# coolbeam/UPFlow_pytorch

Measured on AMD Instinct MI355X. Metric: frame-pairs/sec at 384x1280 bf16, higher is better.
Workload: dtype bf16; 1 GPU; config2: UPFlow_net inference forward (flow fwd+bwd, occlusion masks, SGU on), 384x1280, batch 4 per GPU, random-init weights; global_batch=4, parallelism=replicas x1 (image pairs sharded, no collective), ranks=1, hip_graph=True, capture_fallback=False, steps_in_flight=4, pyramid_convs=HIP (MFMA kernel), pyramid_dtype=fp16

## Files before the change

include/upflow_hip.h:

```cpp
#ifndef UPFLOW_HIP_H
#define UPFLOW_HIP_H

#ifdef __cplusplus
extern "C" {
#endif

enum { UPF_F32 = 0, UPF_F16 = 1, UPF_BF16 = 2 };
enum { UPF_OK = 0, UPF_EINVAL = -1, UPF_EDTYPE = -2, UPF_EALIGN = -3, UPF_EUNSUPPORTED = -4 };
enum { UPF_MASK_NONE = 0, UPF_MASK_LITERAL = 1, UPF_MASK_ROBUST = 2 };

const char* upf_version(void);
const char* upf_last_error(void);

int upf_corr81_forward(const void* f1, const void* f2, void* out,
                       int B, int C, int H, int W, int dtype,
                       long long out_batch_stride, float leaky_slope, void* stream);

int upf_corr81_forward_timed(const void* f1, const void* f2, void* out,
                             int B, int C, int H, int W, int dtype,
                             long long out_batch_stride, float leaky_slope, void* stream,
                             int nrep, float* avg_us, float* min_us);

int upf_corr81_norm_supported(int C, int dtype);
long long upf_corr81_norm_workspace_bytes(int B, int C, int H, int W);
int upf_corr81_norm_forward(const void* f1, const void* f2, void* out,
                            int B, int C, int H, int W, int dtype,
                            long long out_batch_stride, float leaky_slope, void* workspace, void* stream);
int upf_corr81_norm_forward_c8(const void* f1, const void* f2, void* out8, long long out8_batch_stride,
                               int B, int C, int H, int W, int dtype, float leaky_slope, void* workspace, void* stream);
int upf_corr81_norm_forward_pitched(const void* f1, const void* f2, int f_row_pitch, void* out,
                                    int B, int C, int H, int W, int dtype,
                                    long long out_batch_stride, float leaky_slope, void* workspace, void* stream);
int upf_corr81_norm_forward_c8_pitched(const void* f1, const void* f2, int f_row_pitch, void* out8, long long out8_batch_stride,
                                       int B, int C, int H, int W, int dtype, float leaky_slope, void* workspace, void* stream);
int upf_corr81_norm_forward_mixed(const void* f1, const void* f2, int f_row_pitch, void* out,
                                  int B, int C, int H, int W, int dtype, int out_dtype,
                                  long long out_batch_stride, float leaky_slope, void* workspace, void* stream);
int upf_corr81_norm_forward_c8_mixed(const void* f1, const void* f2, int f_row_pitch, void* out8, long long out8_batch_stride,
                                     int B, int C, int H, int W, int dtype, int out_dtype, float leaky_slope, void* workspace, void* stream);
int upf_corr81_norm_forward_timed(const void* f1, const void* f2, void* out,
                                  int B, int C, int H, int W, int dtype,
                                  long long out_batch_stride, float leaky_slope, void* workspace, void* stream,
                                  int nrep, float* avg_us, float* min_us);
int upf_corr81_norm_forward_c8_timed(const void* f1, const void* f2, void* out8, long long out8_batch_stride,
                                     int B, int C, int H, int W, int dtype, float leaky_slope, void* workspace, void* stream,
                                     int nrep, float* avg_us, float* min_us);

int upf_corr81_norm_forward_c8_timed_pitched(const void* f1, const void* f2, int f_row_pitch, void* out8, long long out8_batch_stride,
                                             int B, int C, int H, int W, int dtype, float leaky_slope, void* workspace, void* stream,
                                             int nrep, float* avg_us, float* min_us);

int upf_corr81_norm_forward_c8_timed_mixed(const void* f1, const void* f2, int f_row_pitch, void* out8, long long out8_batch_stride,
                                           int B, int C, int H, int W, int dtype, int out_dtype, float leaky_slope, void* workspace, void* stream,
                                           int nrep, float* avg_us, float* min_us);

int upf_corr_set_option(const char* name, int value);

int upf_corr81_backward(const void* f1, const void* f2, const void* grad_out, void* g1, void* g2,
                        int B, int C, int H, int W, int dtype, void* stream);

int upf_correlation_forward(const void* in1, const void* in2, void* out,
                            int B, int C, int H, int W, int dtype,
                            int pad_size, int kernel_size, int max_displacement,
                            int stride1, int stride2, int corr_type_multiply, void* stream);
int upf_correlation_backward(const void* in1, const void* in2, const void* grad_out, void* g1, void* g2,
                             int B, int C, int H, int W, int dtype,
                             int pad_size, int kernel_size, int max_displacement,
                             int stride1, int stride2, int corr_type_multiply, void* stream);
int upf_correlation_out_shape(int H, int W, int pad_size, int kernel_size, int max_displacement,
                              int stride1, int stride2, int* out_channels, int* out_h, int* out_w);

int upf_warp_forward(const void* x, const float* flow, void* y,
                     int B, int C, int H, int W, int dtype, int mask_mode, int batch_shift, void* stream);
int upf_warp_forward_strided(const void* x, long long x_batch_stride, const float* flow, void* y, long long y_batch_stride,
                             int B, int C, int H, int W, int dtype, int mask_mode, int batch_shift, void* stream);
int upf_warp_forward_pitched(const void* x, long long x_batch_stride, int x_row_pitch, const float* flow, void* y, long long y_batch_stride,
                             int y_row_pitch, int B, int C, int H, int W, int dtype, int mask_mode, int batch_shift, void* stream);
int upf_warp_forward_c8(const void* x8, long long x_batch_stride, const float* flow, void* y8, long long y_batch_stride,
                        int B, int n_oct, int H, int W, int dtype, int mask_mode, int batch_shift, void* stream);
long long upf_warp_backward_workspace_bytes(int B, int C, int H, int W);
int upf_warp_backward(const void* x, const float* flow, const void* grad_y,
                      void* gx, float* gflow, void* workspace,
                      int B, int C, int H, int W, int dtype, int mask_mode, int batch_shift, void* stream);

int upf_flow_upsample_forward(const float* x, float* y, int B, int C, int h, int w, int H, int W,
                              int if_rate, void* stream);
int upf_flow_upsample_backward(const float* grad_y, float* gx, int B, int C, int h, int w, int H, int W,
                               int if_rate, void* stream);

long long upf_sgu_blend_forward_workspace_bytes(int B, int h, int w, int Hf, int Wf);
int upf_sgu_blend_forward(const float* flow_init, const void* x_out, float* flow_up,
                          float* inter_flow, float* inter_mask, void* workspace,
                          int B, int h, int w, int Hf, int Wf, int dtype, void* stream);
int upf_sgu_blend_forward_flow16(const float* flow_init, const void* x_out, float* flow_up, void* flow16, long long flow16_batch_stride,
                                 int flow16_is_c8, int B, int H, int W, int dtype, void* stream);
long long upf_sgu_blend_backward_workspace_bytes(int B, int h, int w, int Hf, int Wf);
int upf_sgu_blend_backward(const float* flow_init, const void* x_out, const float* grad_flow_up,
                           float* g_flow_init32, float* g_x_out32, void* workspace,
                           int B, int h, int w, int Hf, int Wf, int dtype, void* stream);

long long upf_normalize_workspace_bytes(long long N, int HW);
int upf_normalize_forward(const void* x, void* y, float* mean, float* rstd, void* workspace,
                          long long N, int HW, int dtype, void* stream);
int upf_normalize_backward(const void* y, const void* grad_y, const float* rstd, void* gx,
                           long long N, int HW, int dtype, void* stream);

long long upf_conv_packed_bytes(int Cin, int Cout, int kernel_size);
int upf_conv_pack_weights(const void* w , void* w_packed, int Cin, int Cout, int kernel_size,
                          int dtype, void* stream);
int upf_conv_forward(const void* x, long long x_batch_stride, const void* w_packed, const float* bias,
                     void* y, long long y_batch_stride, int B, int Cin, int Cout, int H, int W,
                     int kernel_size, int dilation, int stride, float leaky_slope, int dtype, void* stream);
int upf_conv_forward_pitched(const void* x, long long x_batch_stride, int x_row_pitch, const void* w_packed, const float* bias,
                             void* y, long long y_batch_stride, int y_row_pitch, int B, int Cin, int Cout, int H, int W,
                             int kernel_size, int dilation, int stride, float leaky_slope, int dtype, void* stream);
int upf_conv1x1_forward_mixed(const void* x, long long x_batch_stride, int x_row_pitch, const void* w_packed, const float* bias,
                              void* y, long long y_batch_stride, int y_row_pitch, int y_is_c8, int B, int Cin, int Cout, int H, int W,
                              float leaky_slope, int dtype, int out_dtype, void* stream);
int upf_conv1x1_forward_c8_dual(const void* x, long long x_batch_stride, int x_row_pitch, const void* w_packed, const float* bias,
                                void* y8_a, long long ya_batch_stride, void* y8_b, long long yb_batch_stride,
                                int B, int Cin, int Cout, int H, int W, float leaky_slope, int dtype, int out_dtype, void* stream);
int upf_conv_set_option(const char* name, int value);

long long upf_conv_x3_packed_bytes(int Cin, int Cout, int kernel_size);
int upf_conv_x3_pack_weights(const float* w, void* w_packed, int Cin, int Cout, int kernel_size, void* stream);
int upf_conv_x3_forward(const float* x, long long x_batch_stride, const void* w_packed, const float* bias, float* y,
                        long long y_batch_stride, int B, int Cin, int Cout, int H, int W, int kernel_size, int dilation,
                        int stride, float leaky_slope, int nprod, void* stream);
int upf_conv_x3_set_option(const char* name, int value);
int upf_mfma_f16_denorm_probe(float* out_device, void* stream);

long long upf_conv_packed_bytes_k(int K, int Cout, int kernel_size);
int upf_conv_c8_k(int n8_oct, int C2);
int upf_conv_pack_weights_kmap(const void* w , void* w_packed, int Cin, int Cout, int kernel_size,
                               const int* kmap , int K, int dtype, void* stream);
int upf_conv_forward_c8(const void* x8, long long x8_batch_stride, int n8_oct, const void* x2, long long x2_batch_stride, int C2,
                        const void* w_packed, const float* bias, void* y, long long y_batch_stride, int y_is_c8,
                        int B, int Cout, int H, int W, int kernel_size, int dilation, int stride, float leaky_slope,
                        int dtype, void* stream);
int upf_conv_forward_c8_pitched(const void* x8, long long x8_batch_stride, int n8_oct, const void* x2, long long x2_batch_stride, int x2_row_pitch, int C2,
                                const void* w_packed, const float* bias, void* y, long long y_batch_stride, int y_row_pitch, int y_is_c8,
                                int B, int Cout, int H, int W, int kernel_size, int dilation, int stride, float leaky_slope,
                                int dtype, void* stream);
int upf_conv_c8_set_option(const char* name, int value);
long long upf_conv_packed_bytes_k16(int K, int Cout);
int upf_conv_pack_weights_kmap16(const void* w , void* w_packed, int Cin, int Cout,
                                 const int* kmap , int K, int dtype, void* stream);
int upf_conv_forward_c8_narrow(const void* x8, long long x8_batch_stride, int n8_oct, const void* w_packed16, const float* bias,
                               void* y, long long y_batch_stride, int y_is_c8, int B, int Cout, int H, int W, float leaky_slope,
                               int dtype, void* stream);
int upf_conv_forward_c8_split(const void* x8, long long x8_batch_stride, int n8_oct, const void* w_packed ,
                              const float* bias , void* y8, long long y_batch_stride, int C_main,
                              float* partial, long long partial_batch_stride , int partial_pitch ,
                              int B, int Cout, int H, int W, float leaky_slope, int dtype, void* stream);
int upf_conv_forward_c8_narrow_init(const void* x8, long long x8_batch_stride, int n8_oct, const void* w_packed16,
                                    const float* partial, long long partial_batch_stride, int partial_pitch, int partial_offset ,
                                    void* y, long long y_batch_stride, int y_is_c8, int B, int Cout, int H, int W, float leaky_slope,
                                    int dtype, void* stream);

int upf_conv_pair_forward(const void* x, long long x_batch_stride, int x_row_pitch, int Cin,
                          const void* wa_packed, const float* bias_a , float slope_a, int C1, int stride_a,
                          const void* wb_packed, const float* bias_b , float slope_b, int C2, int stride_b,
                          void* y, long long y_batch_stride, int y_row_pitch, int y_is_c8,
                          int B, int H, int W, int dtype, void* stream);

int upf_conv_pack_weights_f32(const float* w , void* w_packed, int Cin, int Cout, int kernel_size,
                              int dtype, int dgrad, void* stream);
int upf_conv_pack_weights_f32_multi(const float* const* w, void* const* w_packed, const int* Cin, const int* Cout, const int* kernel_size,
                                    const int* dgrad, int njobs, int dtype, void* stream);
int upf_conv_pack_stacked_dgrad(const float* const* w, const int* Cin, const int* Cout, const int* first_channel, int nlayers,
                                void* const* w_packed, const int* slice_channel, const int* slice_width, const int* nconsumers,
                                int nslices, int dtype, void* stream);
int upf_leaky_backward(const void* grad_y, const void* y, void* grad_pre, long long n, float slope, int dtype, void* stream);
int upf_conv_wgrad_supported(int Cin, int Cout, int H, int W, int kernel_size, int dilation, int stride, int dtype);
long long upf_conv_wgrad_workspace_bytes(int B, int Cin, int Cout, int H, int W, int kernel_size, int dilation);
int upf_conv_wgrad(const void* x, long long x_batch_stride, const void* grad_pre, long long g_batch_stride, float* grad_w,
                   void* workspace, int B, int Cin, int Cout, int H, int W, int kernel_size, int dilation, int dtype, void* stream);
typedef struct {
  const void* x;        long long x_batch_stride;
  const void* grad_pre; long long g_batch_stride;
  int B, H, W;
} upf_wgrad_level;
long long upf_conv_wgrad_multi_workspace_bytes(const upf_wgrad_level* levels, int nlevels, int Cin, int Cout, int kernel_size, int dilation);
int upf_conv_wgrad_multi(const upf_wgrad_level* levels , int nlevels, float* grad_w, void* workspace, int Cin, int Cout,
                         int kernel_size, int dilation, int dtype, void* stream);
int upf_conv_wgrad_multi_bias(const upf_wgrad_level* levels, int nlevels, float* grad_w, void* workspace, int Cin, int Cout,
                              int kernel_size, int dilation, const float* const* bias_partials , int npartials, float* grad_bias,
                              int dtype, void* stream);
int upf_space_to_depth2(const void* src, void* dst, int B, int C , int H, int W , int inverse, int dtype, void* stream);
int upf_conv_wgrad_s2d(const upf_wgrad_level* levels, int nlevels, float* grad_w, void* workspace, int Cin, int Cout, int dtype, void* stream);
int upf_act_grad(const void* src, long long src_batch_stride, const void* add, long long add_batch_stride, const void* y,
                 long long y_batch_stride, void* dst, long long dst_batch_stride, float* bias_partial, int B, int C, int HW,
                 float slope, int dtype, void* stream);
int upf_conv_forward_gated(const void* x, long long x_batch_stride, int x_row_pitch, const void* w_packed, const float* bias,
                           void* y, long long y_batch_stride, int y_row_pitch, const void* add, long long add_batch_stride,
                           const void* act, long long act_batch_stride, float mask_slope,
                           int B, int Cin, int Cout, int H, int W, int dtype, void* stream);
int upf_conv_bias_grad_finish(const float* const* partials , int npartials, float* grad_bias,
                              int Cout, void* stream);
long long upf_conv_bias_grad_workspace_bytes(int Cout);
int upf_conv_bias_grad(const void* grad_pre, long long g_batch_stride, float* grad_bias, void* workspace, int B, int Cout, int HW,
                       int dtype, void* stream);

int upf_flow_update(const float* a, const void* b, const void* c, void* out, long long out_batch_stride,
                    int out_is_f32, int N, int per_item, int dtype, void* stream);
int upf_flow_update_c8(const float* a, const void* b, const void* c, void* out8, long long out8_batch_stride,
                       int N, int HW, int dtype, void* stream);

int upf_occ_check(const float* flow_f, const float* flow_b, float* occ_fw, float* occ_bw,
                  int B, int H, int W, float alpha1, float alpha2, void* stream);

int upf_div_selftest(int size, unsigned long long* mismatches, void* stream);

int upf_census_forward(const float* gray1, const float* gray2, float* dist, int B, int H, int W, int max_distance, void* stream);
int upf_census_backward(const float* gray1, const float* gray2, const float* grad_dist, float* g_gray1, float* g_gray2,
                        int B, int H, int W, int max_distance, void* stream);

int upf_boundary_warp_forward(const float* image, const float* flow, const float* start, float* out,
                              int B, int C, int Hi, int Wi, int h, int w, void* stream);
int upf_boundary_warp_backward(const float* image, const float* flow, const float* start, const float* grad_out,
                               float* grad_flow, int B, int C, int Hi, int Wi, int h, int w, void* stream);

int upf_loss_partials(long long n_pixels);

int upf_robust_loss_forward(const float* x, const float* y, const float* occ, float* partials,
                            int B, int C, int HW, float eps, float q, void* stream);
int upf_robust_loss_backward(const float* x, const float* y, const float* occ, const float* coef,
                             float* grad_x, float* grad_y, int B, int C, int HW, float eps, float q, void* stream);

int upf_grey_forward(const float* image, float* grey, int B, int HW, void* stream);

int upf_msd_upup_partials(int B, int H, int W);
int upf_msd_upup_forward(const float* const* x_low, const int* hs, const int* ws, int nlevels, const float* y, const float* occ,
                         float* partials, float* out2, int B, int H, int W, float weight, float eps, float q, void* stream);
int upf_msd_upup_backward(const float* const* x_low, float* const* grad_x_low, const int* hs, const int* ws, int nlevels, const float* y,
                          const float* occ, const float* grad_out, const float* fwd_out2, int B, int H, int W, float weight, float eps, float q,
                          void* stream);

int upf_smooth_edge1_forward(const float* img, const float* pred, float* partials,
                             int B, int Ci, int Cp, int H, int W, void* stream);
int upf_smooth_edge1_backward(const float* img, const float* pred, const float* grad_up, float* grad_pred,
                              int B, int Ci, int Cp, int H, int W, void* stream);

#ifdef __cplusplus
}
#endif
#endif
```

upflow_pytorch_amd/_lib.py:

```python
import ctypes
import os

import torch

_PKG = os.path.dirname(os.path.abspath(__file__))
LIB_PATH = os.environ.get('UPF_HIP_LIB') or os.path.join(_PKG, 'libupflow_hip.so')

UPF_F32, UPF_F16, UPF_BF16 = 0, 1, 2
MASK_NONE, MASK_LITERAL, MASK_ROBUST = 0, 1, 2
_DTYPES = {torch.float32: UPF_F32, torch.float16: UPF_F16, torch.bfloat16: UPF_BF16}

_c = ctypes
_vp, _i, _f, _ll = _c.c_void_p, _c.c_int, _c.c_float, _c.c_longlong

SIGNATURES = {
    'upf_corr81_forward': [_vp, _vp, _vp, _i, _i, _i, _i, _i, _ll, _f, _vp],
    'upf_corr81_forward_timed': [_vp, _vp, _vp, _i, _i, _i, _i, _i, _ll, _f, _vp, _i, _c.POINTER(_f), _c.POINTER(_f)],
    'upf_corr81_norm_forward': [_vp, _vp, _vp, _i, _i, _i, _i, _i, _ll, _f, _vp, _vp],
    'upf_corr81_norm_forward_timed': [_vp, _vp, _vp, _i, _i, _i, _i, _i, _ll, _f, _vp, _vp, _i, _c.POINTER(_f), _c.POINTER(_f)],
    'upf_corr81_norm_forward_c8_timed': [_vp, _vp, _vp, _ll, _i, _i, _i, _i, _i, _f, _vp, _vp, _i, _c.POINTER(_f), _c.POINTER(_f)],
    'upf_corr81_norm_forward_pitched': [_vp, _vp, _i, _vp, _i, _i, _i, _i, _i, _ll, _f, _vp, _vp],
    'upf_corr81_norm_forward_c8_pitched': [_vp, _vp, _i, _vp, _ll, _i, _i, _i, _i, _i, _f, _vp, _vp],
    'upf_corr81_norm_forward_c8_timed_pitched': [_vp, _vp, _i, _vp, _ll, _i, _i, _i, _i, _i, _f, _vp, _vp, _i, _c.POINTER(_f), _c.POINTER(_f)],
    'upf_corr81_norm_forward_c8_timed_mixed': [_vp, _vp, _i, _vp, _ll, _i, _i, _i, _i, _i, _i, _f, _vp, _vp, _i, _c.POINTER(_f), _c.POINTER(_f)],
    'upf_warp_forward_pitched': [_vp, _ll, _i, _vp, _vp, _ll, _i, _i, _i, _i, _i, _i, _i, _i, _vp],
    'upf_conv_forward_gated': [_vp, _ll, _i, _vp, _vp, _vp, _ll, _i, _vp, _ll, _vp, _ll, _f, _i, _i, _i, _i, _i, _i, _vp],
    'upf_conv_forward_pitched': [_vp, _ll, _i, _vp, _vp, _vp, _ll, _i, _i, _i, _i, _i, _i, _i, _i, _i, _f, _i, _vp],
    'upf_conv_forward_c8_pitched': [_vp, _ll, _i, _vp, _ll, _i, _i, _vp, _vp, _vp, _ll, _i, _i, _i, _i, _i, _i, _i, _i, _i, _f, _i, _vp],
    'upf_corr81_norm_forward_mixed': [_vp, _vp, _i, _vp, _i, _i, _i, _i, _i, _i, _ll, _f, _vp, _vp],
    'upf_corr81_norm_forward_c8_mixed': [_vp, _vp, _i, _vp, _ll, _i, _i, _i, _i, _i, _i, _f, _vp, _vp],
    'upf_conv1x1_forward_mixed': [_vp, _ll, _i, _vp, _vp, _vp, _ll, _i, _i, _i, _i, _i, _i, _i, _f, _i, _i, _vp],
    'upf_conv1x1_forward_c8_dual': [_vp, _ll, _i, _vp, _vp, _vp, _ll, _vp, _ll, _i, _i, _i, _i, _i, _f, _i, _i, _vp],
    'upf_corr81_backward': [_vp, _vp, _vp, _vp, _vp, _i, _i, _i, _i, _i, _vp],
    'upf_correlation_forward': [_vp, _vp, _vp, _i, _i, _i, _i, _i, _i, _i, _i, _i, _i, _i, _vp],
    'upf_correlation_backward': [_vp, _vp, _vp, _vp, _vp, _i, _i, _i, _i, _i, _i, _i, _i, _i, _i, _i, _vp],
    'upf_correlation_out_shape': [_i, _i, _i, _i, _i, _i, _i, _c.POINTER(_i), _c.POINTER(_i), _c.POINTER(_i)],
    'upf_warp_forward': [_vp, _vp, _vp, _i, _i, _i, _i, _i, _i, _i, _vp],
    'upf_warp_forward_strided': [_vp, _ll, _vp, _vp, _ll, _i, _i, _i, _i, _i, _i, _i, _vp],
    'upf_warp_forward_c8': [_vp, _ll, _vp, _vp, _ll, _i, _i, _i, _i, _i, _i, _i, _vp],
    'upf_flow_update': [_vp, _vp, _vp, _vp, _ll, _i, _i, _i, _i, _vp],
    'upf_flow_update_c8': [_vp, _vp, _vp, _vp, _ll, _i, _i, _i, _vp],
    'upf_corr81_norm_forward_c8': [_vp, _vp, _vp, _ll, _i, _i, _i, _i, _i, _f, _vp, _vp],
    'upf_warp_backward': [_vp, _vp, _vp, _vp, _vp, _vp, _i, _i, _i, _i, _i, _i, _i, _vp],
    'upf_flow_upsample_forward': [_vp, _vp, _i, _i, _i, _i, _i, _i, _i, _vp],
    'upf_flow_upsample_backward': [_vp, _vp, _i, _i, _i, _i, _i, _i, _i, _vp],
    'upf_sgu_blend_forward': [_vp, _vp, _vp, _vp, _vp, _vp, _i, _i, _i, _i, _i, _i, _vp],
    'upf_sgu_blend_forward_flow16': [_vp, _vp, _vp, _vp, _ll, _i, _i, _i, _i, _i, _vp],
    'upf_sgu_blend_backward': [_vp, _vp, _vp, _vp, _vp, _vp, _i, _i, _i, _i, _i, _i, _vp],
    'upf_normalize_forward': [_vp, _vp, _vp, _vp, _vp, _ll, _i, _i, _vp],
    'upf_normalize_backward': [_vp, _vp, _vp, _vp, _ll, _i, _i, _vp],
    'upf_conv_pack_weights': [_vp, _vp, _i, _i, _i, _i, _vp],
    'upf_conv_forward': [_vp, _ll, _vp, _vp, _vp, _ll, _i, _i, _i, _i, _i, _i, _i, _i, _f, _i, _vp],
    'upf_conv_x3_pack_weights': [_vp, _vp, _i, _i, _i, _vp],
    'upf_conv_x3_forward': [_vp, _ll, _vp, _vp, _vp, _ll, _i, _i, _i, _i, _i, _i, _i, _i, _f, _i, _vp],
    'upf_mfma_f16_denorm_probe': [_vp, _vp],
    'upf_conv_pack_weights_f32': [_vp, _vp, _i, _i, _i, _i, _i, _vp],
    'upf_conv_pack_stacked_dgrad': [_c.POINTER(_vp), _c.POINTER(_i), _c.POINTER(_i), _c.POINTER(_i), _i, _c.POINTER(_vp), _c.POINTER(_i), _c.POINTER(_i), _c.POINTER(_i), _i, _i, _vp],
    'upf_conv_pack_weights_f32_multi': [_c.POINTER(_vp), _c.POINTER(_vp), _c.POINTER(_i), _c.POINTER(_i), _c.POINTER(_i), _c.POINTER(_i), _i, _i, _vp],
    'upf_conv_pack_weights_kmap': [_vp, _vp, _i, _i, _i, _vp, _i, _i, _vp],
    'upf_conv_forward_c8': [_vp, _ll, _i, _vp, _ll, _i, _vp, _vp, _vp, _ll, _i, _i, _i, _i, _i, _i, _i, _i, _f, _i, _vp],
    'upf_conv_pack_weights_kmap16': [_vp, _vp, _i, _i, _vp, _i, _i, _vp],
    'upf_conv_forward_c8_narrow': [_vp, _ll, _i, _vp, _vp, _vp, _ll, _i, _i, _i, _i, _i, _f, _i, _vp],
    'upf_conv_forward_c8_split': [_vp, _ll, _i, _vp, _vp, _vp, _ll, _i, _vp, _ll, _i, _i, _i, _i, _i, _f, _i, _vp],
    'upf_conv_forward_c8_narrow_init': [_vp, _ll, _i, _vp, _vp, _ll, _i, _i, _vp, _ll, _i, _i, _i, _i, _i, _f, _i, _vp],
    'upf_conv_pair_forward': [_vp, _ll, _i, _i, _vp, _vp, _f, _i, _i, _vp, _vp, _f, _i, _i, _vp, _ll, _i, _i, _i, _i, _i, _i, _vp],
    'upf_leaky_backward': [_vp, _vp, _vp, _ll, _f, _i, _vp],
    'upf_conv_wgrad': [_vp, _ll, _vp, _ll, _vp, _vp, _i, _i, _i, _i, _i, _i, _i, _i, _vp],
    'upf_conv_bias_grad': [_vp, _ll, _vp, _vp, _i, _i, _i, _i, _vp],
    'upf_conv_wgrad_multi': [_vp, _i, _vp, _vp, _i, _i, _i, _i, _i, _vp],
    'upf_conv_wgrad_multi_bias': [_vp, _i, _vp, _vp, _i, _i, _i, _i, _vp, _i, _vp, _i, _vp],
    'upf_space_to_depth2': [_vp, _vp, _i, _i, _i, _i, _i, _i, _vp],
    'upf_conv_wgrad_s2d': [_vp, _i, _vp, _vp, _i, _i, _i, _vp],
    'upf_act_grad': [_vp, _ll, _vp, _ll, _vp, _ll, _vp, _ll, _vp, _i, _i, _i, _f, _i, _vp],
    'upf_conv_bias_grad_finish': [_vp, _i, _vp, _i, _vp],
    'upf_census_forward': [_vp, _vp, _vp, _i, _i, _i, _i, _vp],
    'upf_census_backward': [_vp, _vp, _vp, _vp, _vp, _i, _i, _i, _i, _vp],
    'upf_boundary_warp_forward': [_vp, _vp, _vp, _vp, _i, _i, _i, _i, _i, _i, _vp],
    'upf_boundary_warp_backward': [_vp, _vp, _vp, _vp, _vp, _i, _i, _i, _i, _i, _i, _vp],
    'upf_robust_loss_forward': [_vp, _vp, _vp, _vp, _i, _i, _i, _f, _f, _vp],
    'upf_robust_loss_backward': [_vp, _vp, _vp, _vp, _vp, _vp, _i, _i, _i, _f, _f, _vp],
    'upf_grey_forward': [_vp, _vp, _i, _i, _vp],
    'upf_msd_upup_forward': [_vp, _vp, _vp, _i, _vp, _vp, _vp, _vp, _i, _i, _i, _f, _f, _f, _vp],
    'upf_msd_upup_backward': [_vp, _vp, _vp, _vp, _i, _vp, _vp, _vp, _vp, _i, _i, _i, _f, _f, _f, _vp],
    'upf_smooth_edge1_forward': [_vp, _vp, _vp, _i, _i, _i, _i, _i, _vp],
    'upf_smooth_edge1_backward': [_vp, _vp, _vp, _vp, _i, _i, _i, _i, _i, _vp],
    'upf_div_selftest': [_i, _vp, _vp],
    'upf_occ_check': [_vp, _vp, _vp, _vp, _i, _i, _i, _f, _f, _vp],
}



class WgradLevel(_c.Structure):
    _fields_ = [('x', _vp), ('x_batch_stride', _ll), ('grad_pre', _vp), ('g_batch_stride', _ll), ('B', _i), ('H', _i), ('W', _i)]


_lib = None


class UpflowHipError(RuntimeError):
    """Raised for a rejected argument or a failed launch (the reference raises RuntimeError through
    AT_ERROR("CUDA call failed"), correlation_cuda.cc:81-83)."""


def lib():
    global _lib
    if _lib is None:
        if not os.path.exists(LIB_PATH):
            raise UpflowHipError(
                '%s is missing: build it with `python -c "import __graft_entry__ as g; g.build()"` '
                '(hipcc --offload-arch=gfx950). There is no CPU fallback.' % LIB_PATH)
        L = ctypes.CDLL(LIB_PATH)
        for name, argtypes in SIGNATURES.items():
            fn = getattr(L, name)
            fn.argtypes = argtypes
            fn.restype = _i
        L.upf_normalize_workspace_bytes.argtypes = [_ll, _i]
        L.upf_normalize_workspace_bytes.restype = _ll
        L.upf_corr81_norm_supported.argtypes = [_i, _i]
        L.upf_corr81_norm_supported.restype = _i
        L.upf_corr81_norm_workspace_bytes.argtypes = [_i, _i, _i, _i]
        L.upf_corr81_norm_workspace_bytes.restype = _ll
        L.upf_corr_set_option.argtypes = [_c.c_char_p, _i]
        L.upf_corr_set_option.restype = _i
        L.upf_warp_backward_workspace_bytes.argtypes = [_i, _i, _i, _i]
        L.upf_warp_backward_workspace_bytes.restype = _ll
        L.upf_sgu_blend_backward_workspace_bytes.argtypes = [_i, _i, _i, _i, _i]
        L.upf_sgu_blend_backward_workspace_bytes.restype = _ll
        L.upf_sgu_blend_forward_workspace_bytes.argtypes = [_i, _i, _i, _i, _i]
        L.upf_sgu_blend_forward_workspace_bytes.restype = _ll
        L.upf_conv_wgrad_supported.argtypes = [_i] * 8
        L.upf_conv_wgrad_supported.restype = _i
        L.upf_conv_wgrad_workspace_bytes.argtypes = [_i] * 7
        L.upf_conv_wgrad_workspace_bytes.restype = _ll
        L.upf_conv_wgrad_multi_workspace_bytes.argtypes = [_vp, _i, _i, _i, _i, _i]
        L.upf_conv_wgrad_multi_workspace_bytes.restype = _ll
        L.upf_conv_bias_grad_workspace_bytes.argtypes = [_i]
        L.upf_conv_bias_grad_workspace_bytes.restype = _ll
        L.upf_loss_partials.argtypes = [_ll]
        L.upf_loss_partials.restype = _i
        L.upf_msd_upup_partials.argtypes = [_i, _i, _i]
        L.upf_msd_upup_partials.restype = _i
        L.upf_conv_packed_bytes.argtypes = [_i, _i, _i]
        L.upf_conv_packed_bytes.restype = _ll
        L.upf_conv_x3_packed_bytes.argtypes = [_i, _i, _i]
        L.upf_conv_x3_packed_bytes.restype = _ll
        L.upf_conv_set_option.argtypes = [_c.c_char_p, _i]
        L.upf_conv_set_option.restype = _i
        L.upf_conv_c8_set_option.argtypes = [_c.c_char_p, _i]
        L.upf_conv_c8_set_option.restype = _i
        L.upf_conv_x3_set_option.argtypes = [_c.c_char_p, _i]
        L.upf_conv_x3_set_option.restype = _i
        L.upf_conv_packed_bytes_k.argtypes = [_i, _i, _i]
        L.upf_conv_packed_bytes_k.restype = _ll
        L.upf_conv_c8_k.argtypes = [_i, _i]
        L.upf_conv_c8_k.restype = _i
        L.upf_conv_packed_bytes_k16.argtypes = [_i, _i]
        L.upf_conv_packed_bytes_k16.restype = _ll
        L.upf_version.restype = _c.c_char_p
        L.upf_last_error.restype = _c.c_char_p
        _lib = L
        for item in filter(None, os.environ.get('UPF_CONV_OPTS', '').split(',')):
            k, v = item.split('=')
            if L.upf_conv_set_option(k.strip().encode(), int(v)) == -2 ** 31:
                raise UpflowHipError('UPF_CONV_OPTS: unknown option %r' % k)
    return _lib


def version():
    return lib().upf_version().decode()


def dtype_code(t):
    try:
        return _DTYPES[t.dtype]
    except KeyError:
        raise UpflowHipError('unsupported dtype %s (float32 / float16 / bfloat16 only)' % t.dtype)


def check_gpu(*tensors, contiguous=True):
    dev = None
    for t in tensors:
        if t is None:
            continue
        if not t.is_cuda:
            raise UpflowHipError('upflow_pytorch_amd operators run on the GPU only (got a %s tensor); '
                                 'there is no CPU fallback' % t.device)
        if contiguous and not t.is_contiguous():
            raise UpflowHipError('operand must be contiguous NCHW')
        if dev is None:
            dev = t.device
        elif t.device != dev:
            raise UpflowHipError('operands on different devices: %s vs %s' % (dev, t.device))
    return dev


def stream_ptr(device):
    return _vp(torch.cuda.current_stream(device).cuda_stream)


def ptr(t):
    return _vp(t.data_ptr()) if t is not None else _vp(0)


def call(name, *args):
    rc = getattr(lib(), name)(*args)
    if rc != 0:
        raise UpflowHipError('%s failed (%d): %s' % (name, rc, lib().upf_last_error().decode()))
```

upflow_pytorch_amd/csrc/conv_pair.hip:

```cpp
#include "conv_kernel.hpp"

namespace upf {
namespace convp {

using conv::f32x16;
using conv::Mma32;
using conv::u32x2;

constexpr int NT = 256;
template <int SA, int SB, int TH> struct Geo {
  static constexpr int MR = SB * (TH - 1) + 3, MC = SB * 31 + 3;
  static constexpr int XO = (SA == 2) ? 1 : 0;
  static constexpr int IR = SA * (MR - 1) + 3, IC = (SA * (MC - 1) + 3 + XO + 1) / 2 * 2;
};

template <typename T, int K0, int C1O, int TH, bool YC8, int SA, int SB>
__global__ __launch_bounds__(NT, 2)
void conv_pair_kernel(const T* __restrict__ x, long long xbs, int xpitch, int Cin, const T* __restrict__ wa, const float* __restrict__ ba, float slope_a,
                      const T* __restrict__ wb, const float* __restrict__ bb, float slope_b, T* __restrict__ y, long long ybs, int ypitch, int C2,
                      int H, int W, int Hm, int Wm, int Ho, int Wo, int tiles_x, int tiles_y) {
  using G = Geo<SA, SB, TH>;
  constexpr int MR = G::MR, MC = G::MC, IR = G::IR, IC = G::IC, XO = G::XO;
  constexpr bool QUAD = (K0 == 0);
  constexpr int KO = QUAD ? 1 : K0;
  constexpr int NSTEP = QUAD ? 3 : ((K0 == 1) ? 5 : 9);
  constexpr int KSB = C1O / 2;
  constexpr int RPWB = TH / 4;
  extern __shared__ __attribute__((aligned(16))) uint4 lds[];
  uint4* in_s = lds;
  uint4* mid_s = lds + (QUAD ? (IR * IC + 1) / 2 : K0 * IR * IC);

  const int bid = xcd_remap(blockIdx.x, gridDim.x);
  const int tx = bid % tiles_x, ty = (bid / tiles_x) % tiles_y, n = bid / (tiles_x * tiles_y);
  const int x0 = tx * 32, y0 = ty * TH;
  const int my0 = SB * y0 - 1, mx0 = SB * x0 - 1;
  const int tid = threadIdx.x, lane = tid & 63, wave = tid >> 6;
  const int px = lane & 31, kg = lane >> 5;

  {
    const uint32_t plane = (uint32_t)(H * xpitch) * 2u;
    __amdgpu_buffer_rsrc_t xr = __builtin_amdgcn_make_buffer_rsrc(const_cast<T*>(x + (size_t)n * xbs), 0, (uint32_t)Cin * plane, 0x00020000);
    const int iy0 = SA * my0 - 1, ix0 = SA * mx0 - 1 - XO;
    for (int item = tid; item < IR * (IC / 2); item += NT) {
      const int ir = item / (IC / 2), pp = item - ir * (IC / 2);
      const int gy = iy0 + ir, gx = ix0 + 2 * pp;
      const bool in = gy >= 0 && gy < H && gx >= 0 && gx < W;
      const uint32_t off = in ? (uint32_t)(gy * xpitch + gx) * 2u : 0x80000000u;
      const uint32_t hm = (gx + 1 < W) ? 0xffffffffu : 0x0000ffffu;
      if constexpr (QUAD) {
        uint32_t ch[4];
#pragma unroll
        for (int c = 0; c < 4; ++c) ch[c] = __builtin_amdgcn_raw_buffer_load_b32(xr, off + (uint32_t)c * plane, 0, 0) & hm;
        uint2 e0, e1;
        e0.x = __builtin_amdgcn_perm(ch[1], ch[0], 0x05040100u); e1.x = __builtin_amdgcn_perm(ch[1], ch[0], 0x07060302u);
        e0.y = __builtin_amdgcn_perm(ch[3], ch[2], 0x05040100u); e1.y = __builtin_amdgcn_perm(ch[3], ch[2], 0x07060302u);
        uint2* q = reinterpret_cast<uint2*>(in_s);
        q[ir * IC + 2 * pp] = e0;
        q[ir * IC + 2 * pp + 1] = e1;
      }
#pragma unroll
      for (int o = 0; o < K0; ++o) {
        uint32_t ch[8];
#pragma unroll
        for (int c = 0; c < 8; ++c)
          ch[c] = __builtin_amdgcn_raw_buffer_load_b32(xr, off + (uint32_t)(8 * o + c) * plane, 0, 0) & hm;
        uint4 e0, e1;
        e0.x = __builtin_amdgcn_perm(ch[1], ch[0], 0x05040100u); e1.x = __builtin_amdgcn_perm(ch[1], ch[0], 0x07060302u);
        e0.y = __builtin_amdgcn_perm(ch[3], ch[2], 0x05040100u); e1.y = __builtin_amdgcn_perm(ch[3], ch[2], 0x07060302u);
        e0.z = __builtin_amdgcn_perm(ch[5], ch[4], 0x05040100u); e1.z = __builtin_amdgcn_perm(ch[5], ch[4], 0x07060302u);
        e0.w = __builtin_amdgcn_perm(ch[7], ch[6], 0x05040100u); e1.w = __builtin_amdgcn_perm(ch[7], ch[6], 0x07060302u);
        in_s[(o * IR + ir) * IC + 2 * pp] = e0;
        in_s[(o * IR + ir) * IC + 2 * pp + 1] = e1;
      }
    }
  }
  uint4 wA[NSTEP];
#pragma unroll
  for (int s = 0; s < NSTEP; ++s) wA[s] = *reinterpret_cast<const uint4*>(wa + ((size_t)s * 64 + lane) * 8);
  constexpr int C1 = 8 * C1O;
  f32x16 biasA;
#pragma unroll
  for (int e = 0; e < 16; ++e) {
    const int c = (e & 3) + 8 * (e >> 2) + 4 * kg;
    biasA[e] = (c < C1) ? ba[c] : 0.f;
  }
  int offA[NSTEP], offA2[NSTEP];
#pragma unroll
  for (int s = 0; s < NSTEP; ++s) {
    int tap, oct;
    if constexpr (QUAD) { tap = 4 * s + 2 * kg; oct = 0; }
    else if constexpr (K0 == 1) { tap = 2 * s + kg; oct = 0; }
    else { tap = s; oct = kg; }
    const int t1 = tap > 8 ? 8 : tap, t2 = tap + 1 > 8 ? 8 : tap + 1;
    offA[s] = (oct * IR + t1 / 3) * IC + t1 % 3 + XO;
    offA2[s] = (t2 / 3) * IC + t2 % 3 + XO;
  }
  __syncthreads();

  {
    constexpr int NPX = MR * MC, NTILE = (NPX + 31) / 32;
    for (int t = wave; t < NTILE; t += 4) {
      const int p = t * 32 + px;
      const bool pv = p < NPX;
      const int pc = pv ? p : NPX - 1;
      const int mr = pc / MC, mc = pc - mr * MC;
      f32x16 acc = biasA;
      if constexpr (QUAD) {
        const uint2* ib = reinterpret_cast<const uint2*>(in_s) + SA * (mr * IC + mc);
#pragma unroll
        for (int s = 0; s < NSTEP; ++s) {
          const uint2 lo = ib[offA[s]], hi = ib[offA2[s]];
          acc = Mma32<T>::mma(wA[s], make_uint4(lo.x, lo.y, hi.x, hi.y), acc);
        }
      } else {
        const uint4* ib = in_s + SA * (mr * IC + mc);
#pragma unroll
        for (int s = 0; s < NSTEP; ++s) acc = Mma32<T>::mma(wA[s], ib[offA[s]], acc);
      }
      const int my = my0 + mr, mx = mx0 + mc;
      const bool inside = my >= 0 && my < Hm && mx >= 0 && mx < Wm;
      if (pv) {
#pragma unroll
        for (int o = 0; o < C1O; ++o) {
          float v[4];
#pragma unroll
          for (int q = 0; q < 4; ++q) { v[q] = acc[4 * o + q]; v[q] = fmaxf(v[q], v[q] * slope_a); }
          u32x2 w2;
          w2.x = inside ? pack2<T>(v[0], v[1]) : 0u;
          w2.y = inside ? pack2<T>(v[2], v[3]) : 0u;
          *reinterpret_cast<u32x2*>(reinterpret_cast<unsigned char*>(&mid_s[(o * MR + mr) * MC + mc]) + kg * 8) = w2;
        }
      }
    }
  }
  uint4 wB[9][KSB];
#pragma unroll
  for (int tap = 0; tap < 9; ++tap)
#pragma unroll
    for (int ks = 0; ks < KSB; ++ks) wB[tap][ks] = *reinterpret_cast<const uint4*>(wb + ((size_t)(tap * KSB + ks) * 64 + lane) * 8);
  f32x16 acc[RPWB];
#pragma unroll
  for (int e = 0; e < 16; ++e) {
    const int c = (e & 3) + 8 * (e >> 2) + 4 * kg;
    const float bv = (c < C2) ? bb[c] : 0.f;
#pragma unroll
    for (int rr = 0; rr < RPWB; ++rr) acc[rr][e] = bv;
  }
  __syncthreads();

#pragma unroll
  for (int tap = 0; tap < 9; ++tap) {
    const int ky = tap / 3, kx = tap - 3 * ky;
#pragma unroll
    for (int ks = 0; ks < KSB; ++ks)
#pragma unroll
      for (int rr = 0; rr < RPWB; ++rr) {
        const int r = wave * RPWB + rr;
        const uint4 b = mid_s[((2 * ks + kg) * MR + SB * r + ky) * MC + SB * px + kx];
        acc[rr] = Mma32<T>::mma(wB[tap][ks], b, acc[rr]);
      }
  }
  if constexpr (!YC8) {
    if (((ypitch & 7) | (int)(ybs & 7) | (int)(reinterpret_cast<uintptr_t>(y) & 15)) == 0) {
      __syncthreads();
      conv::epilogue_wide<T, RPWB>(acc, reinterpret_cast<unsigned char*>(lds) + wave * conv::EPI_WAVE_BYTES, y + (size_t)n * ybs, C2, Ho, Wo,
                                   0, lane, x0, __builtin_amdgcn_readfirstlane(y0 + wave * RPWB), 1, slope_b, ypitch);
      return;
    }
  }
  const int gx = x0 + px;
#pragma unroll
  for (int rr = 0; rr < RPWB; ++rr) {
    const int gy = y0 + wave * RPWB + rr;
    if (gy >= Ho || gx >= Wo) continue;
    if constexpr (YC8) {
      T* yo = y + (size_t)n * ybs;
#pragma unroll
      for (int g = 0; g < 4; ++g) {
        if (8 * g >= C2) continue;
        float v[4];
#pragma unroll
        for (int q = 0; q < 4; ++q) { v[q] = acc[rr][4 * g + q]; v[q] = fmaxf(v[q], v[q] * slope_b); }
        u32x2 o2;
        o2.x = pack2<T>(v[0], v[1]); o2.y = pack2<T>(v[2], v[3]);
        *reinterpret_cast<u32x2*>(yo + (((size_t)g * Ho + gy) * Wo + gx) * 8 + kg * 4) = o2;
      }
    } else {
      typename Elem<T>::store_t* yo = reinterpret_cast<typename Elem<T>::store_t*>(y + (size_t)n * ybs);
#pragma unroll
      for (int e = 0; e < 16; e += 2) {
        const int c = (e & 3) + 8 * (e >> 2) + 4 * kg;
        float v0 = acc[rr][e], v1 = acc[rr][e + 1];
        v0 = fmaxf(v0, v0 * slope_b); v1 = fmaxf(v1, v1 * slope_b);
        const uint32_t p2 = pack2<T>(v0, v1);
        if (c < C2) yo[((size_t)c * Ho + gy) * ypitch + gx] = (typename Elem<T>::store_t)(p2 & 0xffffu);
        if (c + 1 < C2) yo[((size_t)(c + 1) * Ho + gy) * ypitch + gx] = (typename Elem<T>::store_t)(p2 >> 16);
      }
    }
  }
}

struct PairArgs {
  const void* x; long long xbs; int xpitch, Cin; const void* wa; const float* ba; float slope_a; int C1;
  const void* wb; const float* bb; float slope_b; int C2; void* y; long long ybs; int ypitch; int B, H, W; hipStream_t stream;
  int sa, sb;
};

template <typename T, int K0, int C1O, int TH, bool YC8, int SA, int SB>
int launch_pair(const PairArgs& a) {
  using G = Geo<SA, SB, TH>;
  const int Hm = (a.H - 1) / SA + 1, Wm = (a.W - 1) / SA + 1;
  const int Ho = (Hm - 1) / SB + 1, Wo = (Wm - 1) / SB + 1;
  const int tiles_x = cdiv(Wo, 32), tiles_y = cdiv(Ho, TH);
  const size_t ldsb = (size_t)((K0 == 0 ? (G::IR * G::IC + 1) / 2 : K0 * G::IR * G::IC) + C1O * G::MR * G::MC) * 16;
  static LdsOptIn opt;
  auto kern = &conv_pair_kernel<T, K0, C1O, TH, YC8, SA, SB>;
  opt.ensure(reinterpret_cast<const void*>(kern), ldsb);
  hipLaunchKernelGGL(kern, dim3((unsigned)(a.B * tiles_x * tiles_y)), dim3(NT), ldsb, a.stream, (const T*)a.x, a.xbs, a.xpitch, a.Cin,
                     (const T*)a.wa, a.ba, a.slope_a, (const T*)a.wb, a.bb, a.slope_b, (T*)a.y, a.ybs, a.ypitch, a.C2, a.H, a.W, Hm, Wm, Ho, Wo, tiles_x, tiles_y);
  return check_launch("conv_pair_forward");
}

template <typename T, bool YC8>
int dispatch_pair(const PairArgs& a) {
  const int k0 = a.Cin <= 4 ? 0 : (a.Cin <= 8 ? 1 : 2), c1o = a.C1 / 8;
  if (a.sa == 1) {
    if (k0 == 0 && c1o == 2) return launch_pair<T, 0, 2, 8, YC8, 1, 2>(a);
    if (k0 == 0 && c1o == 4) return launch_pair<T, 0, 4, 4, YC8, 1, 2>(a);
    if (k0 == 1 && c1o == 2 && conv::g_pair_th == 4) return launch_pair<T, 1, 2, 4, YC8, 1, 2>(a);
    if (k0 == 1 && c1o == 2) return launch_pair<T, 1, 2, 8, YC8, 1, 2>(a);
    if (k0 == 1 && c1o == 4) return launch_pair<T, 1, 4, 4, YC8, 1, 2>(a);
    if (k0 == 2 && c1o == 2) return launch_pair<T, 2, 2, 8, YC8, 1, 2>(a);
    return launch_pair<T, 2, 4, 4, YC8, 1, 2>(a);
  }
  if constexpr (!YC8) {
    if (k0 == 0 && c1o == 2) return launch_pair<T, 0, 2, 8, false, 2, 1>(a);
    if (k0 == 0 && c1o == 4) return launch_pair<T, 0, 4, 8, false, 2, 1>(a);
    if (k0 == 1 && c1o == 2 && conv::g_pair_th == 4) return launch_pair<T, 1, 2, 4, false, 2, 1>(a);
    if (k0 == 1 && c1o == 2) return launch_pair<T, 1, 2, 8, false, 2, 1>(a);
    if (k0 == 1 && c1o == 4) return launch_pair<T, 1, 4, 8, false, 2, 1>(a);
    if (k0 == 2 && c1o == 2) return launch_pair<T, 2, 2, 8, false, 2, 1>(a);
    return launch_pair<T, 2, 4, 8, false, 2, 1>(a);
  }
  set_error("conv_pair_forward: [stride 2, stride 1] writes NCHW");
  return UPF_EUNSUPPORTED;
}

}
}

extern "C" int upf_conv_pair_forward(const void* x, long long x_batch_stride, int x_row_pitch, int Cin,
                                     const void* wa_packed, const float* bias_a, float slope_a, int C1, int stride_a,
                                     const void* wb_packed, const float* bias_b, float slope_b, int C2, int stride_b,
                                     void* y, long long y_batch_stride, int y_row_pitch, int y_is_c8,
                                     int B, int H, int W, int dtype, void* stream) {
  using namespace upf;
  UPF_REQUIRE(x && wa_packed && bias_a && wb_packed && bias_b && y, UPF_EINVAL, "conv_pair_forward: null pointer");
  UPF_REQUIRE(B > 0 && H > 0 && W > 0, UPF_EINVAL, "conv_pair_forward: bad shape B=%d H=%d W=%d", B, H, W);
  UPF_REQUIRE(dtype == UPF_BF16 || dtype == UPF_F16, UPF_EDTYPE, "conv_pair_forward: bf16 / fp16 only");
  UPF_REQUIRE(Cin >= 1 && Cin <= 16 && (C1 == 16 || C1 == 32) && C2 >= 1 && C2 <= 32, UPF_EUNSUPPORTED,
              "conv_pair_forward: Cin <= 16, C1 = 16 | 32, C2 <= 32 (got %d, %d, %d)", Cin, C1, C2);
  UPF_REQUIRE((stride_a == 1 && stride_b == 2) || (stride_a == 2 && stride_b == 1), UPF_EUNSUPPORTED,
              "conv_pair_forward: strides (1, 2) or (2, 1), got (%d, %d)", stride_a, stride_b);
  if (x_row_pitch == 0) x_row_pitch = W;
  const int Ho = (H - 1) / 2 + 1, Wo = (W - 1) / 2 + 1;
  if (y_row_pitch == 0) y_row_pitch = Wo;
  UPF_REQUIRE(x_row_pitch >= W && x_row_pitch % 2 == 0 && aligned_to(x, 4) && x_batch_stride % 2 == 0, UPF_EUNSUPPORTED,
              "conv_pair_forward: the input rows are read as pixel pairs: an even row pitch (%d) and a 4-byte aligned base", x_row_pitch);
  UPF_REQUIRE(slope_a >= 0.f && slope_a <= 1.f && slope_b >= 0.f && slope_b <= 1.f, UPF_EINVAL, "conv_pair_forward: leaky slopes in [0,1]");
  UPF_REQUIRE(aligned_to(wa_packed, 16) && aligned_to(wb_packed, 16), UPF_EINVAL, "conv_pair_forward: packed weights must be 16-byte aligned");
  UPF_REQUIRE(y_is_c8 ? (aligned_to(y, 16) && y_batch_stride % 8 == 0) : (y_row_pitch >= Wo), UPF_EINVAL, "conv_pair_forward: bad output layout");
  UPF_REQUIRE((long long)Cin * H * x_row_pitch * 2 < (1ll << 31), UPF_EINVAL, "conv_pair_forward: image too large for one buffer descriptor");
  convp::PairArgs a{x, x_batch_stride, x_row_pitch, Cin, wa_packed, bias_a, slope_a == 0.f ? 1.f : slope_a, C1,
                    wb_packed, bias_b, slope_b == 0.f ? 1.f : slope_b, C2, y, y_batch_stride, y_row_pitch, B, H, W, (hipStream_t)stream, stride_a, stride_b};
  if (dtype == UPF_BF16) return y_is_c8 ? convp::dispatch_pair<bf16_t, true>(a) : convp::dispatch_pair<bf16_t, false>(a);
  return y_is_c8 ? convp::dispatch_pair<f16_t, true>(a) : convp::dispatch_pair<f16_t, false>(a);
}
```

upflow_pytorch_amd/model/pwc_modules.py:

```python
import logging

import torch
import torch.nn as nn
import torch.nn.functional as tf

from .. import ops
from ..utils.tools import tools


def conv(in_planes, out_planes, kernel_size=3, stride=1, dilation=1, isReLU=True, if_IN=False, IN_affine=False, if_BN=False):
    layers = [nn.Conv2d(in_planes, out_planes, kernel_size=kernel_size, stride=stride, dilation=dilation,
                        padding=((kernel_size - 1) * dilation) // 2, bias=True)]
    if isReLU:
        layers.append(nn.LeakyReLU(0.1, inplace=True))
    if if_IN:
        layers.append(nn.InstanceNorm2d(out_planes, affine=IN_affine))
    elif if_BN:
        layers.append(nn.BatchNorm2d(out_planes, affine=IN_affine))
    return nn.Sequential(*layers)


def initialize_msra(modules):
    logging.info("Initializing MSRA")
    for layer in modules:
        if isinstance(layer, (nn.Conv2d, nn.ConvTranspose2d)):
            nn.init.kaiming_normal_(layer.weight)
            if layer.bias is not None:
                nn.init.constant_(layer.bias, 0)


def upsample2d_as(inputs, target_as, mode="bilinear"):
    _, _, h, w = target_as.size()
    return tf.interpolate(inputs, [h, w], mode=mode, align_corners=True)


def _resize_flow(inputs, h, w, mode, if_rate):
    if mode != "bilinear":
        res = tf.interpolate(inputs, [h, w], mode=mode)
        if if_rate:
            _, _, h_, w_ = inputs.size()
            scale = torch.tensor([w / w_, h / h_], dtype=res.dtype, device=res.device).view(1, 2, 1, 1)
            res = res * scale
        return res
    return ops.flow_upsample(inputs, h, w, if_rate)


def upsample2d_flow_as(inputs, target_as, mode="bilinear", if_rate=False):
    _, _, h, w = target_as.size()
    return _resize_flow(inputs, h, w, mode, if_rate)


def upsample_flow(inputs, target_size=None, target_flow=None, mode="bilinear"):
    if target_size is not None:
        h, w = target_size
    elif target_flow is not None:
        _, _, h, w = target_flow.size()
    else:
        raise ValueError('wrong input')
    return _resize_flow(inputs, h, w, mode, True)


def rescale_flow(flow, div_flow, width_im, height_im, to_local=True):
    if to_local:
        u_scale = float(flow.size(3) / width_im / div_flow)
        v_scale = float(flow.size(2) / height_im / div_flow)
    else:
        u_scale = float(width_im * div_flow / flow.size(3))
        v_scale = float(height_im * div_flow / flow.size(2))
    scale = torch.tensor([u_scale, v_scale], dtype=flow.dtype, device=flow.device).view(1, 2, 1, 1)
    return flow * scale


class FeatureExtractor(nn.Module):

    def __init__(self, num_chs, if_end_relu=True, if_end_norm=False):
        super(FeatureExtractor, self).__init__()
        self.num_chs = num_chs
        self.convs = nn.ModuleList(
            nn.Sequential(conv(ci, co, stride=2), conv(co, co, isReLU=if_end_relu, if_IN=if_end_norm))
            for ci, co in zip(num_chs[:-1], num_chs[1:]))

    def forward(self, x, outs=None, pitched=False):
        pyramid = []
        cache = self.__dict__.setdefault('_fast_cache', {})
        hip = getattr(self, 'hip_convs', True)
        for i, stage in enumerate(self.convs):
            if (hip and FUSE_PAIRS[0] and not getattr(self, '_no_fuse_pairs', False) and len(stage[0]) == 2 and len(stage[1]) == 2
                    and ops.conv_pair_supported(x, stage[0][0], stage[1][0])):
                pc = cache.get(('pair', i)) or cache.setdefault(('pair', i), _PackedConvPair(stage[0], stage[1]))
                ho, wo = ops.conv3x3_out_hw(x.shape[2], x.shape[3], 2)
                y = outs[i] if (outs is not None and outs[i] is not None) else ops.empty_nchw((x.shape[0], stage[1][0].out_channels, ho, wo), x.dtype, x.device, pitched=pitched)
                x = pc(x, y)
                pyramid.append(x)
                continue
            x = fast_conv_seq(stage[0], x, cache, allow_hip=hip, pitched=pitched)
            x = fast_conv_seq(stage[1], x, cache, out=None if outs is None else outs[i], allow_hip=hip, pitched=pitched)
            pyramid.append(x)
        return pyramid[::-1]

    def out_shapes(self, H, W):
        shapes = []
        for c in self.num_chs[1:]:
            H, W = (H - 1) // 2 + 1, (W - 1) // 2 + 1
            shapes.append((c, H, W))
        return shapes


class WarpingLayer_no_div(nn.Module):

    def __init__(self, mask_mode='literal'):
        super(WarpingLayer_no_div, self).__init__()
        self.mask_mode = mask_mode

    def forward(self, x, flow, batch_shift=0):
        return ops.warp(x, flow, self.mask_mode, batch_shift)


class WarpingLayer(nn.Module):

    def __init__(self, mask_mode='literal'):
        super(WarpingLayer, self).__init__()
        self.mask_mode = mask_mode

    def forward(self, x, flow, height_im, width_im, div_flow):
        H, W = x.shape[2:]
        sx = (W - 1) / max(width_im - 1, 1) / div_flow
        sy = (H - 1) / max(height_im - 1, 1) / div_flow
        scale = torch.tensor([sx, sy], dtype=torch.float32, device=flow.device).view(1, 2, 1, 1)
        return ops.warp(x, flow.float() * scale, self.mask_mode)


class _PackedConv3x3(object):

    def __init__(self, seq):
        self.conv = seq[0]
        self.slope = 0.1 if any(isinstance(m, nn.LeakyReLU) for m in seq) else 0.0
        self.key = None
        self.packed = None
        self.bias = None
        self.key32 = None
        self.packed32 = None

    def _key(self):
        w, b = self.conv.weight, self.conv.bias
        return (w._version, w.dtype, w.device, w.data_ptr(), b._version, b.data_ptr())

    def get(self):
        key = self._key()
        if key != self.key:
            self.packed = ops.conv3x3_pack(self.conv.weight)
            self.bias = self.conv.bias.detach().float().contiguous()
            self.key = key
        return self.packed, self.bias

    def get32(self):
        key = self._key()
        if key != self.key32:
            self.packed32 = ops.conv3x3_pack(self.conv.weight.detach().float())
            self.bias = self.conv.bias.detach().float().contiguous()
            self.key32 = key
        return self.packed32, self.bias

    def invalidate(self):
        self.key = None
        self.key32 = None

    def __call__(self, x_view, y_view):
        c = self.conv
        if x_view.dtype != torch.float32 and x_view.shape[3] < 8:
            packed, bias = self.get32()
            ho, wo = ops.conv3x3_out_hw(x_view.shape[2], x_view.shape[3], c.stride[0])
            yf = torch.empty((x_view.shape[0], c.out_channels, ho, wo), dtype=torch.float32, device=x_view.device)
            ops.conv3x3_forward_raw(x_view.float(), packed, bias, yf, c.dilation[0], self.slope, c.stride[0], c.kernel_size[0])
            y_view.copy_(yf)
            return y_view
        packed, bias = self.get()
        return ops.conv3x3_forward_raw(x_view, packed, bias, y_view, c.dilation[0], self.slope, c.stride[0], c.kernel_size[0])


def packed_convs(net):
    out = []
    for m in net.modules():
        d = m.__dict__
        out += list(d.get('_fast_cache', {}).values())
        out += list(d.get('_packed', None) or [])
        for v in d.get('_packed8', {}).values():
            out += list(v[0]) if isinstance(v, tuple) else list(v)
    return [pc for pc in out if hasattr(pc, 'invalidate')]


def packed_operands(net):
    ts = []
    for pc in packed_convs(net):
        ts += [t for t in (getattr(pc, 'packed', None), getattr(pc, 'packed32', None), getattr(pc, 'bias', None)) if torch.is_tensor(t)]
        ts += [t for t in getattr(pc, 'extra_operands', lambda: [])() if torch.is_tensor(t)]
    return ts


_NO_NARROW = [False]


class _PackedConvC8(object):

    def __init__(self, seq, c8_channels=(), tail_channels=()):
        self.conv = seq[0]
        self.slope = 0.1 if any(isinstance(m, nn.LeakyReLU) for m in seq) else 0.0
        self.maps = (tuple(c8_channels), tuple(tail_channels))
        self.narrow = (not _NO_NARROW[0]) and ops.conv_c8_narrow_ok(self.conv.out_channels, self.conv.kernel_size[0], self.conv.dilation[0],
                                                                    self.conv.stride[0], len(self.maps[1]) > 0) and len(self.maps[0]) > 0
        self.key = None
        self.packed = None
        self.bias = None

    def get(self):
        w, b = self.conv.weight, self.conv.bias
        key = (w._version, w.dtype, w.device, w.data_ptr(), b._version, b.data_ptr())
        if key != self.key:
            self.packed = ops.conv_c8_pack16(w, self.maps[0]) if self.narrow else ops.conv_c8_pack(w, self.maps[0], self.maps[1])
            self.bias = self.conv.bias.detach().float().contiguous()
            self.key = key
        return self.packed, self.bias

    def invalidate(self):
        self.key = None

    def dual(self, x2, y_a, y_b):
        packed, bias = self.get()
        c = self.conv
        p = ops.nchw_pitch(x2)
        if (DUAL_1X1[0] and c.kernel_size == (1, 1) and not self.narrow and c.out_channels <= 32 and p is not None and p % 8 == 0
                and x2.data_ptr() % 16 == 0 and x2.stride(0) % 8 == 0):
            return ops.conv1x1_c8_dual_raw(x2, packed, bias, y_a, y_b, self.slope)
        self(None, x2, y_a)
        return self(None, x2, y_b)

    def __call__(self, x8, x2, y):
        packed, bias = self.get()
        if self.narrow:
            return ops.conv_c8_forward_narrow_raw(x8, packed, bias, y, self.slope)
        return ops.conv_c8_forward_raw(x8, x2, packed, bias, y, self.conv.dilation[0], self.slope, self.conv.kernel_size[0], self.conv.stride[0])


class _PackedTailC8(object):

    def __init__(self, seqs, m, J, kmap):
        self.m, self.J = int(m), sorted(int(j) for j in J)
        self.kmap = list(kmap)
        self.main = seqs[m][0]
        self.convs = [seqs[m][0]] + [seqs[j][0] for j in self.J]
        self.widths = [q[0].out_channels for q in seqs]
        self.slopes = {j: (0.1 if any(isinstance(m_, nn.LeakyReLU) for m_ in seqs[j]) else 0.0) for j in [m] + self.J}
        self.cmain = self.main.out_channels
        self.cin = self.main.in_channels
        self.offsets, off = {}, 0
        for j in self.J:
            self.offsets[j] = off
            off += (self.widths[j] + 3) // 4 * 4
        self.pp = off
        self.cout = self.cmain + off
        self.key = None
        self.packed = self.bias = None
        self.finish = {}

    @staticmethod
    def plan(widths):
        n = len(widths)
        cin = [None] * n
        acc = 0
        for k in range(n):
            cin[k] = acc
            acc += widths[k]
        best, best_score = None, 0
        for m in range(n - 2, -1, -1):
            if widths[m] % 8:
                continue
            mt = (widths[m] + 31) // 32
            free = 32 * (4 if mt >= 3 else mt) - widths[m]
            if mt > 4:
                continue
            J, used = [], 0
            for j in range(n - 1, m, -1):
                need = (widths[j] + 3) // 4 * 4
                if widths[j] > 16 or used + need > free or (j < n - 1 and widths[j] % 8):
                    break
                J.append(j); used += need
            if not J or any(widths[k] % 8 for k in range(m, n - 1)):
                continue
            score = len(J) * (cin[m] + 1000)
            if score > best_score:
                best, best_score = (m, sorted(J)), score
        return best

    def _key(self):
        k = []
        for c in self.convs:
            k += [c.weight._version, c.weight.dtype, c.weight.device, c.weight.data_ptr(), c.bias._version, c.bias.data_ptr()]
        return tuple(k)

    def get(self):
        key = self._key()
        if key != self.key:
            c0 = self.main
            rows, bias = [c0.weight.detach()], [c0.bias.detach().float()]
            self.finish = {}
            for j, c in zip(self.J, self.convs[1:]):
                front = sum(self.widths[self.m:j])
                w = c.weight.detach()
                assert w.shape[1] == front + self.cin
                pad = (c.out_channels + 3) // 4 * 4 - c.out_channels
                rows.append(w[:, front:])
                bias.append(c.bias.detach().float())
                if pad:
                    rows.append(w.new_zeros((pad, self.cin) + tuple(w.shape[2:])))
                    bias.append(bias[0].new_zeros(pad))
                self.finish[j] = ops.conv_c8_pack16(w[:, :front].contiguous(), list(range(front)))
            self.packed = ops.conv_c8_pack(torch.cat(rows, 0).contiguous(), self.kmap)
            self.bias = torch.cat(bias).contiguous()
            self.key = key
        return self.packed, self.bias

    def extra_operands(self):
        return list(self.finish.values())

    def invalidate(self):
        self.key = None

    def main_pass(self, x8, y8):
        packed, bias = self.get()
        B, _, H, W, _ = x8.shape
        part = torch.empty((B, self.pp // 4, H, W, 4), dtype=torch.float32, device=x8.device)
        ops.conv_c8_forward_split_raw(x8, packed, bias, y8, part, self.slopes[self.m])
        return part

    def finish_pass(self, j, x8_front, part, y):
        self.get()
        return ops.conv_c8_forward_narrow_init_raw(x8_front, self.finish[j], part, self.offsets[j], self.widths[j], y, self.slopes[j])


class _PackedConvPair(object):

    def __init__(self, seq_a, seq_b):
        self.convs = (seq_a[0], seq_b[0])
        self.strides = (seq_a[0].stride[0], seq_b[0].stride[0])
        self.slopes = tuple(0.1 if any(isinstance(m_, nn.LeakyReLU) for m_ in q) else 0.0 for q in (seq_a, seq_b))
        self.key = None
        self.packed = self.packed_b = self.bias = self.bias_b = None

    def _key(self):
        k = []
        for c in self.convs:
            k += [c.weight._version, c.weight.dtype, c.weight.device, c.weight.data_ptr(), c.bias._version, c.bias.data_ptr()]
        return tuple(k)

    def get(self):
        key = self._key()
        if key != self.key:
            a, b = self.convs
            self.packed, self.packed_b = ops.conv_pair_pack(a.weight, b.weight)
            self.bias, self.bias_b = a.bias.detach().float().contiguous(), b.bias.detach().float().contiguous()
            self.key = key
        return self.packed, self.bias, self.packed_b, self.bias_b

    def extra_operands(self):
        return [self.packed_b, self.bias_b]

    def invalidate(self):
        self.key = None

    def __call__(self, x, y):
        pa, ba, pb, bb = self.get()
        return ops.conv_pair_forward_raw(x, pa, ba, self.slopes[0], pb, bb, self.slopes[1], y, self.strides)


DUAL_1X1 = [True]
FUSE_PAIRS = [True]
MERGE_TAIL = [True]


def c8_level_ok(nb, H, W, dtype):
    return dtype in (torch.bfloat16, torch.float16) and nb * ((W + 31) // 32) * ((H + 7) // 8) >= 200


def fast_conv_seq(seq, x, cache, out=None, allow_hip=True, pitched=False):
    c = seq[0]
    k = c.kernel_size[0]
    if (allow_hip and _fast_conv_ok(x) and c.kernel_size in ((3, 3), (1, 1)) and c.stride[0] == c.stride[1] and c.groups == 1 and len(seq) <= 2
            and c.padding == (((k - 1) * c.dilation[0]) // 2,) * 2
            and (ops.conv3x3_supported(x, c.out_channels, c.dilation[0], c.stride[0], k)
                 or (x.shape[3] < 8 and 1 <= c.dilation[0] <= 16 and (c.stride[0] == 1 or (c.stride[0] == 2 and c.dilation[0] == 1 and k == 3))))):
        pc = cache.get(id(seq))
        if pc is None:
            pc = cache[id(seq)] = _PackedConv3x3(seq)
        ho, wo = ops.conv3x3_out_hw(x.shape[2], x.shape[3], c.stride[0])
        y = out if out is not None else ops.empty_nchw((x.shape[0], c.out_channels, ho, wo), x.dtype, x.device, pitched=pitched)
        return pc(x, y)
    if torch.is_grad_enabled() and x.is_cuda and x.dtype in (torch.bfloat16, torch.float16) and c.weight.dtype == torch.float32:
        y = train_conv_seq(seq, x)
    else:
        y = seq(x if x.is_contiguous() else x.contiguous())
    if out is not None:
        out.copy_(y)
        return out
    return y


def train_conv_seq(seq, x):
    c = seq[0]
    k = c.kernel_size[0]
    slope = 0.0
    for m in list(seq)[1:]:
        if isinstance(m, nn.LeakyReLU):
            slope = float(m.negative_slope)
        else:
            return seq(x.float()).to(x.dtype)
    if (c.kernel_size in ((3, 3), (1, 1)) and c.stride[0] == c.stride[1] and c.groups == 1 and c.padding == (((k - 1) * c.dilation[0]) // 2,) * 2
            and ops.conv_train_supported(x, c.weight, c.stride[0], c.dilation[0])):
        return ops.conv_train(x, c.weight, c.bias, c.dilation[0], slope, c.stride[0])
    return seq(x.float()).to(x.dtype)


FP32_CONV = ['hip_x3']
FP32_CONV_NPROD = {'hip_x3': 3, 'hip_x3s': 11}


class fp32_conv_mode(object):
    def __init__(self, mode):
        if mode != 'miopen' and mode not in FP32_CONV_NPROD:
            raise ValueError("fp32_conv must be one of %s or 'miopen', got %r" % (sorted(FP32_CONV_NPROD), mode))
        self.mode = mode

    def __enter__(self):
        self.saved = (FP32_CONV[0], ops.CONV_X3_NPROD[0])
        FP32_CONV[0] = self.mode
        ops.CONV_X3_NPROD[0] = FP32_CONV_NPROD.get(self.mode, ops.CONV_X3_NPROD[0])

    def __exit__(self, *exc):
        FP32_CONV[0], ops.CONV_X3_NPROD[0] = self.saved


def _fast_conv_ok(t):
    if torch.is_grad_enabled() or not t.is_cuda:
        return False
    if t.dtype == torch.float32:
        return FP32_CONV[0] != 'miopen'
    return t.dtype in (torch.bfloat16, torch.float16)


class _DenseStack(tools.abstract_model):
    _NAMES = ('conv1', 'conv2', 'conv3', 'conv4', 'conv5')

    def _build(self, ch_in, f_channels, out_channel):
        n = ch_in
        for i, f in enumerate(f_channels):
            setattr(self, 'conv%d' % (i + 1), conv(n, f))
            n += f
        self.conv_last = conv(n, out_channel, isReLU=False)
        self._ch_in, self._f, self._n_total = ch_in, tuple(f_channels), n
        self._packed = None
        return n

    def alloc_buffer(self, B, H, W, dtype, device, tail=0):
        buf = torch.empty((B, self._n_total + tail, H, W), dtype=dtype, device=device)
        x0 = self._n_total - self._ch_in
        return buf, buf[:, x0:self._n_total]

    def forward_in_buffer(self, buf, out=None):
        if self._packed is None:
            self._packed = [_PackedConv3x3(getattr(self, n)) for n in self._NAMES] + [_PackedConv3x3(self.conv_last)]
        nt = self._n_total
        hi = nt - self._ch_in
        for pc, f in zip(self._packed[:5], self._f):
            pc(buf[:, hi:nt], buf[:, hi - f:hi])
            hi -= f
        x5 = buf[:, :nt]
        if out is None:
            out = torch.empty((buf.shape[0], self.conv_last[0].out_channels) + tuple(buf.shape[2:]), dtype=buf.dtype, device=buf.device)
        self._packed[5](x5, out)
        return x5, out

    def c8_ok(self):
        return self._ch_in % 8 == 0 and all(f % 8 == 0 for f in self._f)

    def c8_outputs_ok(self):
        return all(f % 8 == 0 for f in self._f)

    def forward_in_buffer_c8(self, buf8, out=None, in_map=None):
        key = None if in_map is None else tuple(in_map)
        cache = self.__dict__.setdefault('_packed8', {})
        if key not in cache:
            imap = list(range(self._ch_in)) if in_map is None else list(in_map)
            assert len(imap) % 8 == 0 and sorted(m for m in imap if m >= 0) == list(range(self._ch_in)), 'in_map must place every input channel once'
            packed, nconv = [], 0
            for name, f in zip(self._NAMES, self._f):
                packed.append(_PackedConvC8(getattr(self, name), list(range(nconv)) + [m + nconv if m >= 0 else -1 for m in imap]))
                nconv += f
            packed.append(_PackedConvC8(self.conv_last, list(range(nconv)) + [m + nconv if m >= 0 else -1 for m in imap]))
            widths = list(self._f) + [self.conv_last[0].out_channels]
            seqs = [getattr(self, n_) for n_ in self._NAMES] + [self.conv_last]
            plain = all(all(isinstance(x_, (nn.Conv2d, nn.LeakyReLU)) for x_ in q_) for q_ in seqs)
            pl = _PackedTailC8.plan(widths) if plain else None
            if pl is not None:
                nbefore = sum(self._f[:pl[0]])
                packed.append(_PackedTailC8(seqs, pl[0], pl[1], list(range(nbefore)) + [q + nbefore if q >= 0 else -1 for q in imap]))
            cache[key] = (packed, len(imap) // 8)
        packed, n_in = cache[key]
        nl = len(self._f)
        no = sum(self._f) // 8 + n_in
        starts, hi = [], sum(self._f) // 8
        for f in self._f:
            starts.append(hi)
            hi -= f // 8
        starts.append(hi)
        if out is None:
            out = torch.empty((buf8.shape[0], self.conv_last[0].out_channels) + tuple(buf8.shape[2:4]), dtype=buf8.dtype, device=buf8.device)
        tail = packed[nl + 1] if (len(packed) > nl + 1 and MERGE_TAIL[0] and not getattr(self, '_no_merge_tail', False)) else None
        part = None
        for k in range(nl + 1):
            y = buf8[:, starts[k + 1]:starts[k]] if k < nl else out
            if tail is not None and k == tail.m:
                part = tail.main_pass(buf8[:, starts[k]:no], y)
            elif tail is not None and k in tail.J:
                tail.finish_pass(k, buf8[:, starts[k]:starts[tail.m]], part, y)
            else:
                packed[k](buf8[:, starts[k]:no], None, y)
        return out

    def _train_convs(self):
        seqs = [getattr(self, n) for n in self._NAMES] + [self.conv_last]
        slope = None
        for i, q in enumerate(seqs):
            act = list(q)[1:]
            if i < 5:
                if len(act) != 1 or not isinstance(act[0], nn.LeakyReLU):
                    return None, None
                slope = float(act[0].negative_slope)
            elif act:
                return None, None
        return [q[0] for q in seqs], slope

    def train_in_buffer_ok(self, inputs):
        convs, _ = self._train_convs()
        return convs is not None and not getattr(self, '_no_train_buffer', False) and ops.dense_stack_train_supported(inputs, convs)

    def forward_train(self, inputs, flow_tail=None):
        convs, slope = self._train_convs()
        return ops.dense_stack_train(inputs, convs, slope, flow_tail)

    def forward(self, x):
        if _fast_conv_ok(x):
            buf, slot = self.alloc_buffer(x.shape[0], x.shape[2], x.shape[3], x.dtype, x.device)
            slot.copy_(x)
            return self.forward_in_buffer(buf)
        if self.train_in_buffer_ok([x]):
            buf, out = self.forward_train([x])
            return buf, out
        cache = self.__dict__.setdefault('_fast_cache', {})
        for name in self._NAMES:
            x = torch.cat([fast_conv_seq(getattr(self, name), x, cache), x], dim=1)
        return x, fast_conv_seq(self.conv_last, x, cache)


class FlowEstimatorDense_v2(_DenseStack):
    def __init__(self, ch_in, f_channels=(128, 128, 96, 64, 32), out_channel=2):
        super(FlowEstimatorDense_v2, self).__init__()
        self.n_channels = self._build(ch_in, f_channels, out_channel)


class FlowEstimatorDense(FlowEstimatorDense_v2):

    def __init__(self, ch_in):
        super(FlowEstimatorDense, self).__init__(ch_in)


class OpticalFlowEstimator(nn.Module):

    def __init__(self, ch_in):
        super(OpticalFlowEstimator, self).__init__()
        self.convs = nn.Sequential(conv(ch_in, 128), conv(128, 128), conv(128, 96), conv(96, 64), conv(64, 32))
        self.conv_last = conv(32, 2, isReLU=False)

    def forward(self, x):
        x_intm = self.convs(x)
        return x_intm, self.conv_last(x_intm)


class ContextNetwork_v2_(nn.Module):

    def __init__(self, ch_in, f_channels=(128, 128, 128, 96, 64, 32, 2)):
        super(ContextNetwork_v2_, self).__init__()
        dil = (1, 2, 4, 8, 16, 1, 1)
        chans = (ch_in,) + tuple(f_channels)
        self.convs = nn.Sequential(*[conv(chans[i], chans[i + 1], 3, 1, dil[i], isReLU=(i < 6)) for i in range(7)])

    def forward(self, x):
        cache = self.__dict__.setdefault('_fast_cache', {})
        for seq in self.convs:
            x = fast_conv_seq(seq, x, cache)
        return x

    def forward_c8(self, x, in_map=None):
        key = None if in_map is None else tuple(in_map)
        cache = self.__dict__.setdefault('_packed8', {})
        if key not in cache:
            chans = [s_[0].in_channels for s_ in self.convs]
            first = _PackedConvC8(self.convs[0], (), range(chans[0])) if in_map is None else _PackedConvC8(self.convs[0], list(in_map))
            cache[key] = [first] + [_PackedConvC8(self.convs[i], range(chans[i])) for i in range(1, 7)]
        B, H, W = x.shape[0], x.shape[2], x.shape[3]
        t = None
        for i, pc in enumerate(cache[key]):
            co = self.convs[i][0].out_channels
            y = ops.c8_empty(B, co, H, W, x.dtype, x.device) if i < 6 else torch.empty((B, co, H, W), dtype=x.dtype, device=x.device)
            if i == 0:
                pc(x if in_map is not None else None, None if in_map is not None else x, y)
            else:
                pc(t, None, y)
            t = y
        return t


class ContextNetwork(ContextNetwork_v2_):

    def __init__(self, ch_in):
        super(ContextNetwork, self).__init__(ch_in)
```

upflow_pytorch_amd/model/upflow.py:

```python
import os
import torch
import torch.nn as nn
import torch.nn.functional as F

from .. import ops
from ..utils.tools import tools
from ..utils.loss import loss_functions
from .pwc_modules import (conv, initialize_msra, upsample2d_flow_as, upsample_flow, FlowEstimatorDense_v2,
                          ContextNetwork_v2_, WarpingLayer_no_div, FeatureExtractor, _DenseStack, _fast_conv_ok,
                          fast_conv_seq, c8_level_ok, _PackedConvC8)
from .correlation_package.correlation import Correlation


FLOW16_IN_BLEND = [True]


class network_tools():
    class sgu_model(tools.abstract_model):

        def __init__(self, mask_mode='literal'):
            super(network_tools.sgu_model, self).__init__()

            class FlowEstimatorDense_temp(_DenseStack):
                def __init__(self, ch_in, f_channels=(128, 128, 96, 64, 32), ch_out=2):
                    super(FlowEstimatorDense_temp, self).__init__()
                    self.num_feature_channel = self._build(ch_in, f_channels, ch_out)

            self.warping_layer = WarpingLayer_no_div(mask_mode)
            self.dense_estimator_mask = FlowEstimatorDense_temp(64, f_channels=(32, 32, 32, 16, 8), ch_out=3)
            self.upsample_output_conv = nn.Sequential(conv(3, 16, kernel_size=3, stride=1, dilation=1),
                                                      conv(16, 16, stride=2),
                                                      conv(16, 32, kernel_size=3, stride=1, dilation=1),
                                                      conv(32, 32, stride=2), )

        def forward(self, flow_init, feature_1, feature_2, output_level_flow=None, batch_shift=0):
            if flow_init.shape[2:] != feature_1.shape[2:]:
                flow_init = upsample2d_flow_as(flow_init, feature_1, mode="bilinear", if_rate=True)
            feature_2_warp = self.warping_layer(feature_2, flow_init, batch_shift)
            est = self.dense_estimator_mask
            if _fast_conv_ok(feature_1):
                buf, slot = est.alloc_buffer(feature_1.shape[0], feature_1.shape[2], feature_1.shape[3], feature_1.dtype, feature_1.device)
                slot[:, :feature_1.shape[1]] = feature_1
                slot[:, feature_1.shape[1]:] = feature_2_warp
                _, x_out = est.forward_in_buffer(buf)
            else:
                _, x_out = est(torch.cat((feature_1, feature_2_warp), dim=1))
            return ops.sgu_blend(flow_init, x_out, output_level_flow)

        def forward_in_buffer(self, flow_init, buf, slot, output_level_flow=None, batch_shift=0, flow16=None):
            c1 = slot.shape[1] // 2
            ops.warp_into(slot[:, :c1], flow_init, slot[:, c1:], self.warping_layer.mask_mode, batch_shift)
            _, x_out = self.dense_estimator_mask.forward_in_buffer(buf)
            if flow16 is not None:
                return flow_init, ops.sgu_blend_flow16(flow_init, x_out, flow16), None, None
            return ops.sgu_blend(flow_init, x_out, output_level_flow, want_inter=False)

        def forward_in_buffer_c8(self, flow_init, buf8, output_level_flow=None, batch_shift=0, tap=None, flow16=None):
            est = self.dense_estimator_mask
            o0 = (est._n_total - est._ch_in) // 8
            half = est._ch_in // 16
            ops.warp_c8_into(buf8[:, o0:o0 + half], flow_init, buf8[:, o0 + half:o0 + 2 * half], self.warping_layer.mask_mode, batch_shift)
            x_out = est.forward_in_buffer_c8(buf8)
            if tap is not None:
                tap('sgu_x_out', x_out)
            if flow16 is not None:
                return flow_init, ops.sgu_blend_flow16(flow_init, x_out, flow16), None, None
            return ops.sgu_blend(flow_init, x_out, output_level_flow, want_inter=False)

        def output_conv(self, x, out=None, out8=None, pitched=False):
            cache = self.__dict__.setdefault('_fast_cache', {})
            n = len(self.upsample_output_conv)
            from . import pwc_modules as _pm
            if n == 4 and _pm.FUSE_PAIRS[0] and not getattr(self, '_no_fuse_pairs', False) and all(len(q) == 2 for q in self.upsample_output_conv):
                sq = self.upsample_output_conv
                if ops.conv_pair_supported(x, sq[0][0], sq[1][0]):
                    B_, _, H_, W_ = x.shape
                    h1, w1 = ops.conv3x3_out_hw(H_, W_, 2)
                    mid = ops.empty_nchw((B_, sq[1][0].out_channels, h1, w1), x.dtype, x.device, pitched=True)
                    if ops.conv_pair_supported(mid, sq[2][0], sq[3][0]):
                        pa = cache.get('pair01') or cache.setdefault('pair01', _pm._PackedConvPair(sq[0], sq[1]))
                        pb = cache.get('pair23') or cache.setdefault('pair23', _pm._PackedConvPair(sq[2], sq[3]))
                        pa(x, mid)
                        h2, w2 = ops.conv3x3_out_hw(h1, w1, 2)
                        if out8 is not None:
                            return pb(mid, out8)
                        y = out if out is not None else ops.empty_nchw((B_, sq[3][0].out_channels, h2, w2), x.dtype, x.device, pitched=pitched)
                        return pb(mid, y)
            for i, seq in enumerate(self.upsample_output_conv):
                if i == n - 1 and out8 is not None:
                    pc = cache.get('c8_last')
                    if pc is None:
                        pc = cache['c8_last'] = _PackedConvC8(seq, (), range(seq[0].in_channels))
                    return pc(None, x, out8)
                x = fast_conv_seq(seq, x, cache, out=out if i == n - 1 else None, pitched=pitched)
            return x

    @classmethod
    def normalize_features(cls, feature_list, normalize, center, moments_across_channels=True, moments_across_images=True):
        if normalize and center and not moments_across_channels and not moments_across_images:
            return [ops.normalize(f) for f in feature_list]
        axes = [1, 2, 3] if moments_across_channels else [2, 3]
        means = [torch.mean(f.float(), dim=axes, keepdim=True) for f in feature_list]
        vars_ = [torch.var(f.float(), dim=axes, keepdim=True) for f in feature_list]
        if moments_across_images:
            means = [torch.mean(torch.stack(means, dim=0), dim=(0,))] * len(feature_list)
            vars_ = [torch.var(torch.stack(vars_, dim=0), dim=(0,))] * len(feature_list)
        stds = [torch.sqrt(v + 1e-16) for v in vars_]
        out = list(feature_list)
        if center:
            out = [f - m.to(f.dtype) for f, m in zip(out, means)]
        if normalize:
            out = [f / s.to(f.dtype) for f, s in zip(out, stds)]
        return out

    @classmethod
    def edge_aware_smoothness_order1(cls, img, pred):
        return ops.smooth_edge1(img, pred)

    @classmethod
    def edge_aware_smoothness_order2(cls, img, pred):
        def dx(t, s=1):
            return t[:, :, :-s, :] - t[:, :, s:, :]

        def dy(t, s=1):
            return t[:, :, :, :-s] - t[:, :, :, s:]
        wx = torch.exp(-dx(img, 2).abs().mean(1, keepdim=True))
        wy = torch.exp(-dy(img, 2).abs().mean(1, keepdim=True))
        return (dx(dx(pred)).abs() * wx).mean() + (dy(dy(pred)).abs() * wy).mean()

    @classmethod
    def flow_smooth_delta(cls, flow, if_second_order=False):
        return loss_functions.flow_smooth_delta(flow, if_second_order)

    @classmethod
    def weighted_ssim(cls, x, y, weight, c1=float('inf'), c2=9e-6, weight_epsilon=0.01):
        if c1 == float('inf') and c2 == float('inf'):
            raise ValueError('Both c1 and c2 are infinite, SSIM loss is zero. This is likely unintended.')

        def pool(z):
            return F.avg_pool2d(z, (3, 3), (1, 1))
        w_avg = pool(weight)
        w_eps = weight + weight_epsilon
        inv = 1.0 / (w_avg + weight_epsilon)

        def wpool(z):
            return pool(z * w_eps) * inv
        mu_x, mu_y = wpool(x), wpool(y)
        sigma_x = wpool(x ** 2) - mu_x ** 2
        sigma_y = wpool(y ** 2) - mu_y ** 2
        sigma_xy = wpool(x * y) - mu_x * mu_y
        if c1 == float('inf'):
            n, d = (2 * sigma_xy + c2), (sigma_x + sigma_y + c2)
        elif c2 == float('inf'):
            n, d = 2 * mu_x * mu_y + c1, mu_x ** 2 + mu_y ** 2 + c1
        else:
            n = (2 * mu_x * mu_y + c1) * (2 * sigma_xy + c2)
            d = (mu_x ** 2 + mu_y ** 2 + c1) * (sigma_x + sigma_y + c2)
        return torch.clamp((1 - n / d) / 2, 0, 1), w_avg

    @classmethod
    def photo_loss_multi_type(cls, x, y, occ_mask, photo_loss_type='abs_robust', photo_loss_delta=0.4, photo_loss_use_occ=False):
        occ_weight = occ_mask
        if photo_loss_type == 'abs_robust':
            s, s_occ = ops.robust_loss_sums(x, y, occ_mask if photo_loss_use_occ else None, q=photo_loss_delta, eps=0.01)
            return s / (s_occ + 1e-6) if photo_loss_use_occ else s / float(x.numel())
        elif photo_loss_type == 'charbonnier':
            loss_diff = ((x - y) ** 2 + 1e-6).pow(photo_loss_delta)
        elif photo_loss_type == 'L1':
            loss_diff = (x - y + 1e-6).abs()
        elif photo_loss_type == 'SSIM':
            loss_diff, occ_weight = cls.weighted_ssim(x, y, occ_mask)
        else:
            raise ValueError('wrong photo_loss type: %s' % photo_loss_type)
        if photo_loss_use_occ:
            return torch.sum(loss_diff * occ_weight) / (torch.sum(occ_weight) + 1e-6)
        return torch.mean(loss_diff)


class UPFlow_net(tools.abstract_model):
    class config(tools.abstract_config):
        def __init__(self):
            self.occ_type = 'for_back_check'
            self.alpha_1 = 0.1
            self.alpha_2 = 0.5
            self.occ_check_obj_out_all = 'obj'
            self.stop_occ_gradient = False
            self.smooth_level = 'final'
            self.smooth_type = 'edge'
            self.smooth_order_1_weight = 1
            self.smooth_order_2_weight = 0
            self.photo_loss_type = 'abs_robust'
            self.photo_loss_delta = 0.4
            self.photo_loss_use_occ = False
            self.photo_loss_census_weight = 0
            self.if_norm_before_cost_volume = False
            self.norm_moments_across_channels = True
            self.norm_moments_across_images = True
            self.multi_scale_distillation_weight = 0
            self.multi_scale_distillation_style = 'upup'
            self.multi_scale_distillation_occ = True
            self.if_froze_pwc = False
            self.input_or_sp_input = 1
            self.if_use_boundary_warp = True
            self.if_sgu_upsample = False
            self.if_use_cor_pytorch = False
            self.warp_mask_mode = 'literal'
            self.hip_pyramid_convs = True
            self.train_conv_dtype = 'fp32'
            self.fp32_conv = 'hip_x3'
            self.fp16_overflow_check = False

        def __call__(self, ):
            return UPFlow_net(self)

    def __init__(self, conf: config):
        super(UPFlow_net, self).__init__()
        self.conf = conf
        if conf.if_use_cor_pytorch:
            raise ops.UpflowHipError(
                "if_use_cor_pytorch=True selects the reference's CPU fallback (utils/pytorch_correlation.py); "
                "this package has no CPU path — its restatement lives in oracle/ as test infrastructure")
        self.search_range = 4
        self.num_chs = [3, 16, 32, 64, 96, 128, 196]
        self.estimator_f_channels = (128, 128, 96, 64, 32)
        self.context_f_channels = (128, 128, 128, 96, 64, 32, 2)
        self.output_level = 4
        self.num_levels = 7
        self.leakyRELU = nn.LeakyReLU(0.1, inplace=True)
        self.feature_pyramid_extractor = FeatureExtractor(self.num_chs)
        self.feature_pyramid_extractor.hip_convs = bool(getattr(conf, 'hip_pyramid_convs', True))
        self.warping_layer = WarpingLayer_no_div(conf.warp_mask_mode)
        self.dim_corr = (self.search_range * 2 + 1) ** 2
        self.num_ch_in = self.dim_corr + 32 + 2
        self.flow_estimators = FlowEstimatorDense_v2(self.num_ch_in, f_channels=self.estimator_f_channels)
        self.context_networks = ContextNetwork_v2_(self.flow_estimators.n_channels + 2, f_channels=self.context_f_channels)
        self.conv_1x1 = nn.ModuleList([conv(c, 32, kernel_size=1, stride=1, dilation=1) for c in (196, 128, 96, 64, 32)])
        self.correlation = Correlation(pad_size=self.search_range, kernel_size=1, max_displacement=self.search_range,
                                       stride1=1, stride2=1, corr_multiply=1)
        self.sgi_model = network_tools.sgu_model(conf.warp_mask_mode) if conf.if_sgu_upsample else None
        self.occ_check_model = tools.occ_check_model(occ_type=conf.occ_type, occ_alpha_1=conf.alpha_1,
                                                     occ_alpha_2=conf.alpha_2, obj_out_all=conf.occ_check_obj_out_all)
        initialize_msra(self.modules())
        if conf.if_froze_pwc:
            self.froze_PWC()

    def forward(self, input_dict: dict):
        im1_ori, im2_ori = input_dict['im1'], input_dict['im2']
        if input_dict['if_loss'] and self.conf.input_or_sp_input != 1:
            im1, im2 = input_dict['im1_sp'], input_dict['im2_sp']
        else:
            im1, im2 = im1_ori, im2_ori
        flow_f, flow_b, flows = self.forward_2_frame_v3(im1, im2, if_loss=input_dict['if_loss'])
        occ_fw, occ_bw = self.occ_check_model(flow_f=flow_f, flow_b=flow_b)
        out = {'flow_f_out': flow_f, 'flow_b_out': flow_b, 'occ_fw': occ_fw, 'occ_bw': occ_bw}
        if getattr(self.conf, 'fp16_overflow_check', False) and not torch.cuda.is_current_stream_capturing():
            if not (bool(torch.isfinite(flow_f).all()) and bool(torch.isfinite(flow_b).all())):
                raise ops.UpflowHipError('non-finite flow: an fp16 feature / activation overflowed (|x| > 65504) — run this input in '
                                         'bfloat16 (net.to_inference(torch.bfloat16)) or fp32')
        if input_dict['if_loss']:
            self._losses(input_dict, out, flows, im1_ori.float(), im2_ori.float())
        return out

    def _losses(self, input_dict, out, flows, im1, im2):
        c = self.conf
        nt = network_tools
        flow_f, flow_b, occ_fw, occ_bw = out['flow_f_out'], out['flow_b_out'], out['occ_fw'], out['occ_bw']
        if c.smooth_level == 'final':
            s_f, s_b, s_im1, s_im2 = flow_f, flow_b, im1, im2
        elif c.smooth_level == '1/4':
            s_f, s_b = flows[0]
            s_im1 = F.interpolate(im1, s_f.shape[2:], mode='area')
            s_im2 = F.interpolate(im2, s_f.shape[2:], mode='area')
        else:
            raise ValueError('wrong smooth level choosed: %s' % c.smooth_level)
        smooth = 0
        for order, weight in ((1, c.smooth_order_1_weight), (2, c.smooth_order_2_weight)):
            if weight <= 0:
                continue
            if c.smooth_type == 'edge':
                fn = nt.edge_aware_smoothness_order1 if order == 1 else nt.edge_aware_smoothness_order2
                smooth = smooth + weight * fn(img=s_im1, pred=s_f) + weight * fn(img=s_im2, pred=s_b)
            elif c.smooth_type == 'delta':
                smooth = smooth + weight * nt.flow_smooth_delta(s_f, order == 2) + weight * nt.flow_smooth_delta(s_b, order == 2)
            else:
                raise ValueError('wrong smooth_type: %s' % c.smooth_type)
        out['smooth_loss'] = smooth
        if c.if_use_boundary_warp:
            im1_s, im2_s, start = input_dict['im1_raw'].float(), input_dict['im2_raw'].float(), input_dict['start']
            im1_warp = tools.boundary_dilated_warp.warp_im(im2_s, flow_f, start)
            im2_warp = tools.boundary_dilated_warp.warp_im(im1_s, flow_b, start)
        else:
            im1_warp = tools.torch_warp(im2, flow_f)
            im2_warp = tools.torch_warp(im1, flow_b)
        if c.stop_occ_gradient:
            occ_fw, occ_bw = occ_fw.clone().detach(), occ_bw.clone().detach()
        kw = dict(photo_loss_type=c.photo_loss_type, photo_loss_delta=c.photo_loss_delta, photo_loss_use_occ=c.photo_loss_use_occ)
        out['photo_loss'] = nt.photo_loss_multi_type(im1, im1_warp, occ_fw, **kw) + nt.photo_loss_multi_type(im2, im2_warp, occ_bw, **kw)
        out['im1_warp'], out['im2_warp'] = im1_warp, im2_warp
        if c.photo_loss_census_weight > 0:
            ckw = dict(q=c.photo_loss_delta, charbonnier_or_abs_robust=False, if_use_occ=c.photo_loss_use_occ, averge=True)
            census = loss_functions.census_loss_torch(img1=im1, img1_warp=im1_warp, mask=occ_fw, **ckw) + \
                loss_functions.census_loss_torch(img1=im2, img1_warp=im2_warp, mask=occ_bw, **ckw)
            out['census_loss'] = census * c.photo_loss_census_weight
        else:
            out['census_loss'] = None
        if c.multi_scale_distillation_weight > 0:
            label_f, label_b = flow_f.detach(), flow_b.detach()
            lv_f, lv_b = [f for f, _ in flows], [b for _, b in flows]
            if (c.multi_scale_distillation_style == 'upup' and not getattr(self, '_no_fused_msd', False) and not os.environ.get('UPF_NO_FUSED_MSD') and hasattr(ops, 'msd_upup_supported')
                    and ops.msd_upup_supported(label_f, lv_f) and ops.msd_upup_supported(label_b, lv_b)):
                use = c.multi_scale_distillation_occ
                out['msd_loss'] = (ops.msd_upup_loss(lv_f, label_f, occ_fw if use else None, c.multi_scale_distillation_weight)
                                   + ops.msd_upup_loss(lv_b, label_b, occ_bw if use else None, c.multi_scale_distillation_weight))
                return
            label_f, label_b = label_f.clone(), label_b.clone()
            terms = []
            for lvl_f, lvl_b in flows:
                if c.multi_scale_distillation_style == 'down':
                    tf_, tb_ = upsample_flow(label_f, target_flow=lvl_f), upsample_flow(label_b, target_flow=lvl_b)
                    of_ = F.interpolate(occ_fw, lvl_f.shape[2:], mode='nearest')
                    ob_ = F.interpolate(occ_bw, lvl_b.shape[2:], mode='nearest')
                elif c.multi_scale_distillation_style == 'upup':
                    tf_, tb_, of_, ob_ = label_f, label_b, occ_fw, occ_bw
                    lvl_f, lvl_b = upsample_flow(lvl_f, target_flow=label_f), upsample_flow(lvl_b, target_flow=label_b)
                else:
                    raise ValueError('wrong multi_scale_distillation_style: %s' % c.multi_scale_distillation_style)
                mkw = dict(photo_loss_type='abs_robust', photo_loss_use_occ=c.multi_scale_distillation_occ)
                terms.append(nt.photo_loss_multi_type(x=lvl_f, y=tf_, occ_mask=of_, **mkw))
                terms.append(nt.photo_loss_multi_type(x=lvl_b, y=tb_, occ_mask=ob_, **mkw))
            out['msd_loss'] = c.multi_scale_distillation_weight * sum(terms)
        else:
            out['msd_loss'] = None

    def forward_2_frame_v3(self, x1_raw, x2_raw, if_loss=False):
        cdt = self.feature_pyramid_extractor.convs[0][0][0].weight.dtype
        from .pwc_modules import fp32_conv_mode
        with fp32_conv_mode(getattr(self.conf, 'fp32_conv', 'hip_x3')):
            return self._forward_2_frame_v3(x1_raw, x2_raw, if_loss, cdt)

    def _forward_2_frame_v3(self, x1_raw, x2_raw, if_loss, cdt):
        if not torch.is_grad_enabled() or getattr(self, 'stacked_training', True):
            B = x1_raw.shape[0]
            X = ops.empty_nchw((2 * B,) + tuple(x1_raw.shape[1:]), cdt, x1_raw.device,
                               pitched=self._pitched() and not torch.is_grad_enabled() and x1_raw.is_cuda)
            X[:B].copy_(x1_raw)
            X[B:].copy_(x2_raw)
            ddt = self.flow_estimators.conv1[0].weight.dtype
            if ddt != cdt:
                if torch.is_grad_enabled() or not x1_raw.is_cuda or ddt == torch.float32 or cdt == torch.float32:
                    raise ops.UpflowHipError('pyramid_dtype: 16-bit GPU inference only')
                Xd = ops.empty_nchw(tuple(X.shape), ddt, X.device, pitched=self._pitched())
                Xd[:B].copy_(x1_raw)
                Xd[B:].copy_(x2_raw)
                return self._forward_stacked(X, B, frames_dec=Xd)
            tdt = {'bf16': torch.bfloat16, 'fp16': torch.float16}.get(getattr(self.conf, 'train_conv_dtype', 'fp32'))
            if tdt is not None and torch.is_grad_enabled() and cdt == torch.float32:
                convs = [m for m in self.modules() if isinstance(m, nn.Conv2d)] if getattr(self, 'shared_grad_sinks', True) else []
                with ops.shared_conv_grads(convs):
                    return self._forward_stacked(X.to(tdt), B, tdt)
            return self._forward_stacked(X, B)
        x1_raw = x1_raw.to(cdt)
        x2_raw = x2_raw.to(cdt)
        x1_pyramid = self.feature_pyramid_extractor(x1_raw)
        x2_pyramid = self.feature_pyramid_extractor(x2_raw)
        B, _, h0, w0 = x1_pyramid[0].shape
        flow_f = torch.zeros(B, 2, h0, w0, dtype=torch.float32, device=x1_raw.device)
        flow_b = torch.zeros_like(flow_f)
        flows = []
        for level in range(self.output_level + 1):
            x1, x2 = x1_pyramid[level], x2_pyramid[level]
            flow_f, flow_b, res_f, res_b = self.decode_level_res(
                level=level, flow_1=flow_f, flow_2=flow_b, feature_1=x1, feature_1_1x1=self.conv_1x1[level](x1),
                feature_2=x2, feature_2_1x1=self.conv_1x1[level](x2), img_ori_1=x1_raw, img_ori_2=x2_raw)
            flow_f = flow_f + res_f
            flow_b = flow_b + res_b
            flows.append([flow_f, flow_b])
        flow_f_out = upsample2d_flow_as(flow_f, x1_raw, mode="bilinear", if_rate=True)
        flow_b_out = upsample2d_flow_as(flow_b, x1_raw, mode="bilinear", if_rate=True)
        if self.conf.if_sgu_upsample:
            g1 = self.sgi_model.output_conv(x1_raw)
            g2 = self.sgi_model.output_conv(x2_raw)
            flow_f_out = self.self_guided_upsample(flow_up_bilinear=flow_f, feature_1=g1, feature_2=g2, output_level_flow=flow_f_out)
            flow_b_out = self.self_guided_upsample(flow_up_bilinear=flow_b, feature_1=g2, feature_2=g1, output_level_flow=flow_b_out)
        return flow_f_out, flow_b_out, flows[::-1]

    def _forward_stacked(self, X, B, train_dtype=None, frames_dec=None):

        if (_fast_conv_ok(X) and X.dtype != torch.float32 and self.conf.if_norm_before_cost_volume and not self.conf.norm_moments_across_channels
                and not self.conf.norm_moments_across_images and not getattr(self, '_no_fast_stacked', False)
                and self.feature_pyramid_extractor.out_shapes(X.shape[2], X.shape[3])[-1][2] >= 8):
            return self._forward_stacked_fast(X, B, frames_dec)
        ddt = None if frames_dec is None else frames_dec.dtype
        pyramid = self.feature_pyramid_extractor(X)
        h0, w0 = pyramid[0].shape[2:]
        flow = torch.zeros(2 * B, 2, h0, w0, dtype=torch.float32, device=X.device)
        sgu = self.conf.if_sgu_upsample
        flows = []
        for level in range(self.output_level + 1):
            Fm = pyramid[level]
            A = fast_conv_seq(self.conv_1x1[level], Fm, self.__dict__.setdefault('_fast_cache', {}))
            if ddt is not None:
                A = A.to(ddt)
            flow_up = upsample2d_flow_as(flow, Fm, mode="bilinear", if_rate=True)
            if level == 0:
                Fw = torch.roll(Fm, shifts=B, dims=0)
            else:
                if sgu:
                    flow_up = self.sgi_model(flow_up, A, A, batch_shift=B)[1]
                Fw = self.warping_layer(Fm, flow_up, batch_shift=B)
            if self.conf.if_norm_before_cost_volume:
                kw = dict(normalize=True, center=True, moments_across_channels=self.conf.norm_moments_across_channels,
                          moments_across_images=self.conf.norm_moments_across_images)
                if self.conf.norm_moments_across_images:
                    n1, n2w = network_tools.normalize_features((Fm[:B], Fw[:B]), **kw)
                    n2, n1w = network_tools.normalize_features((Fm[B:], Fw[B:]), **kw)
                    Fn, Fwn = torch.cat([n1, n2], 0), torch.cat([n2w, n1w], 0)
                else:
                    Fn, Fwn = network_tools.normalize_features((Fm, Fw), **kw)
            else:
                Fn, Fwn = Fm, Fw
            if ddt is not None:
                Fn, Fwn = Fn.to(ddt), Fwn.to(ddt)
            flow = self._level_update(Fn, Fwn, A, flow_up, add_to_flow=True)
            flows.append(list(ops.split_batch(flow, B)))
        flow_out = upsample2d_flow_as(flow, X, mode="bilinear", if_rate=True)
        if sgu:
            G = self.sgi_model.output_conv(X if ddt is None else frames_dec)
            flow_out = self.sgi_model(flow, G, G, output_level_flow=flow_out, batch_shift=B)[1]
        f_out, b_out = ops.split_batch(flow_out, B)
        return f_out, b_out, flows[::-1]

    def _pitched(self):
        return not getattr(self, '_no_pitch', False)

    def _tap(self, name, t):
        taps = getattr(self, '_taps', None)
        if taps is not None:
            taps.append((name, t))

    def _forward_stacked_fast(self, X, B, frames_dec=None):
        nb = 2 * B
        dev, pdt = X.device, X.dtype
        dt = pdt if frames_dec is None else frames_dec.dtype
        cache = self.__dict__.setdefault('_fast_cache', {})
        fpe, est, sgi = self.feature_pyramid_extractor, self.flow_estimators, self.sgi_model
        sgu = self.conf.if_sgu_upsample
        nlev = self.output_level + 1
        nc = self.dim_corr
        shapes = fpe.out_shapes(X.shape[2], X.shape[3])[::-1]
        pit = self._pitched()
        pairs = [ops.empty_nchw((2, nb) + shp, pdt, dev, pitched=pit) for shp in shapes[:nlev]]
        outs = ([p[0] for p in pairs] + [None] * (len(shapes) - nlev))[::-1]
        pyramid = fpe(X, outs=outs, pitched=pit)
        self._tap('X', X)
        for i_, p_ in enumerate(pyramid):
            self._tap('pyramid%d' % i_, p_)
        flow = torch.zeros((nb, 2) + shapes[0][1:], dtype=torch.float32, device=dev)
        flows = []
        for level in range(nlev):
            Fm, pair = pyramid[level], pairs[level]
            C, H, W = shapes[level]
            use_sgu = sgu and level > 0
            c8 = c8_level_ok(nb, H, W, dt) and (W % 8 == 0 or (pit and W >= 8)) and not getattr(self, '_no_c8', False)
            c8_est = (c8 and level > 0 and est.c8_outputs_ok() and not getattr(self, '_no_c8_est', False)
                      and ops.corr81_norm_supported(pair) and not getattr(self, '_no_fused_norm', False) and nc == 81
                      and est._ch_in == nc + 32 + 2 and self.conv_1x1[level][0].out_channels == 32
                      and self.context_networks.convs[0][0].in_channels == est._n_total + 2)
            if c8_est:
                flow, flows_entry = self._level_c8(level, Fm, pair, flow, nb, B, C, H, W, dt, dev, cache, use_sgu)
                flows.append(flows_entry)
                self._tap('L%d.flow' % level, flow)
                continue
            buf, slot = est.alloc_buffer(nb, H, W, dt, dev, tail=2)
            sbuf8 = None
            if use_sgu and c8 and sgi.dense_estimator_mask.c8_ok() and not getattr(self, '_no_c8_sgu', False):
                em = sgi.dense_estimator_mask
                sbuf8 = ops.c8_empty(nb, em._n_total, H, W, dt, dev)
                o0 = (em._n_total - em._ch_in) // 8
                pc = cache.get(('c8_1x1', level))
                if pc is None:
                    pc = cache[('c8_1x1', level)] = _PackedConvC8(self.conv_1x1[level], (), range(C))
                pc(None, Fm, sbuf8[:, o0:o0 + 4])
                fast_conv_seq(self.conv_1x1[level], Fm, cache, out=slot[:, nc:nc + 32])
            elif use_sgu:
                sbuf, sslot = sgi.dense_estimator_mask.alloc_buffer(nb, H, W, dt, dev)
                A = fast_conv_seq(self.conv_1x1[level], Fm, cache, out=sslot[:, :32])
                slot[:, nc:nc + 32].copy_(A)
            else:
                fast_conv_seq(self.conv_1x1[level], Fm, cache, out=slot[:, nc:nc + 32])
            flow_up = flow if (level == 0 and tuple(flow.shape[2:]) == (H, W)) else upsample2d_flow_as(flow, Fm, mode="bilinear", if_rate=True)
            f16 = None
            if level == 0:
                pair[1, :B].copy_(Fm[B:])
                pair[1, B:].copy_(Fm[:B])
            else:
                f16 = slot[:, nc + 32:] if (use_sgu and FLOW16_IN_BLEND[0]) else None
                if sbuf8 is not None:
                    flow_up = sgi.forward_in_buffer_c8(flow_up, sbuf8, batch_shift=B, flow16=f16)[1]
                elif use_sgu:
                    flow_up = sgi.forward_in_buffer(flow_up, sbuf, sslot, batch_shift=B, flow16=f16)[1]
                ops.warp_into(Fm, flow_up, pair[1], self.warping_layer.mask_mode, B)
            if ops.corr81_norm_supported(pair) and not getattr(self, '_no_fused_norm', False):
                ops.corr81_norm_forward_raw(pair[0], pair[1], out=slot[:, :nc], leaky_slope=0.1)
            else:
                normed = ops.normalize(pair.reshape(2 * nb, C, H, W))
                ops.corr81_forward_raw(normed[:nb], normed[nb:], out=slot[:, :nc], leaky_slope=0.1)
            if f16 is None:
                ops.flow_update(flow_up, out=slot[:, nc + 32:])
            _, res = est.forward_in_buffer(buf)
            ops.flow_update(flow_up, res, out=buf[:, est._n_total:])
            fine = self.context_networks.forward_c8(buf) if (c8 and W % 8 == 0 and not getattr(self, '_no_c8_ctx', False)) else self.context_networks(buf)
            flow = ops.flow_update(flow_up, res, fine)
            flows.append([flow[:B], flow[B:]])
            self._tap('L%d.pair' % level, pair)
            self._tap('L%d.buf' % level, buf)
            self._tap('L%d.flow_up' % level, flow_up)
            self._tap('L%d.res' % level, res)
            self._tap('L%d.fine' % level, fine)
            self._tap('L%d.flow' % level, flow)
        flow_out = upsample2d_flow_as(flow, X, mode="bilinear", if_rate=True)
        self._tap('final.flow_bilinear', flow_out)
        if sgu:
            guide = self._final_guidance(X if frames_dec is None else frames_dec, nb, tuple(flow.shape[2:]))
            if guide[0] == 'c8':
                flow_out = sgi.forward_in_buffer_c8(flow, guide[1], output_level_flow=flow_out, batch_shift=B)[1]
            else:
                flow_out = sgi.forward_in_buffer(flow, guide[1], guide[2], output_level_flow=flow_out, batch_shift=B)[1]
        return flow_out[:B], flow_out[B:], flows[::-1]

    def _final_guidance(self, X, nb, hw4):
        sgi = self.sgi_model
        em = sgi.dense_estimator_mask
        H4, W4 = hw4
        dt, dev = X.dtype, X.device
        last = sgi.upsample_output_conv[-1][0]
        hw = (X.shape[2], X.shape[3])
        for seq_ in sgi.upsample_output_conv:
            hw = ops.conv3x3_out_hw(hw[0], hw[1], seq_[0].stride[0])
        pit = self._pitched()
        w_last = ops.conv3x3_out_hw(X.shape[2], X.shape[3], sgi.upsample_output_conv[1][0].stride[0])[1]
        if (c8_level_ok(nb, H4, W4, dt) and not getattr(self, '_no_c8', False) and not getattr(self, '_no_c8_sgu', False) and em.c8_ok()
                and (w_last % 8 == 0 or (pit and w_last >= 8))
                and last.stride[0] == 2 and last.in_channels > 16 and last.out_channels == em._ch_in // 2 and hw == (H4, W4)):
            sbuf8 = ops.c8_empty(nb, em._n_total, H4, W4, dt, dev)
            o0 = (em._n_total - em._ch_in) // 8
            sgi.output_conv(X, out8=sbuf8[:, o0:o0 + em._ch_in // 16], pitched=pit)
            return ('c8', sbuf8)
        sbuf, sslot = em.alloc_buffer(nb, H4, W4, dt, dev)
        G = sgi.output_conv(X, out=sslot[:, :32], pitched=pit)
        if tuple(G.shape[2:]) != (H4, W4):
            raise RuntimeError('sgu output_conv / flow size mismatch %s vs %s' % (tuple(G.shape), (H4, W4)))
        return ('nchw', sbuf, sslot)

    def _level_c8(self, level, Fm, pair, flow, nb, B, C, H, W, dt, dev, cache, use_sgu):
        est, sgi = self.flow_estimators, self.sgi_model
        nconv = sum(est._f) // 8
        ncorr = ops.CORR81_C8_OCTETS
        in_map = ops.corr81_c8_channel_map() + list(range(81, 113)) + [113, 114] + [-1] * 6
        n_est = nconv + len(in_map) // 8
        buf8 = ops.c8_empty(nb, (n_est + 1) * 8, H, W, dt, dev)
        o_feat, o_flow = nconv + ncorr, nconv + ncorr + 4
        pc = cache.get(('c8_1x1', level))
        if pc is None:
            pc = cache[('c8_1x1', level)] = _PackedConvC8(self.conv_1x1[level], (), range(C))
        if use_sgu:
            em = sgi.dense_estimator_mask
            sbuf8 = ops.c8_empty(nb, em._n_total, H, W, dt, dev)
            o0 = (em._n_total - em._ch_in) // 8
            pc.dual(Fm, buf8[:, o_feat:o_feat + 4], sbuf8[:, o0:o0 + 4])
        else:
            pc(None, Fm, buf8[:, o_feat:o_feat + 4])
        flow_up = upsample2d_flow_as(flow, Fm, mode="bilinear", if_rate=True)
        self._tap('L%d.flow_bilinear' % level, flow_up)
        if use_sgu:
            f16 = buf8[:, o_flow:o_flow + 1] if FLOW16_IN_BLEND[0] else None
            flow_up = sgi.forward_in_buffer_c8(flow_up, sbuf8, batch_shift=B, tap=lambda n_, t_: self._tap('L%d.%s' % (level, n_), t_), flow16=f16)[1]
            self._tap('L%d.sbuf8' % level, sbuf8)
            self._tap('L%d.flow_sgu' % level, flow_up)
        ops.warp_into(Fm, flow_up, pair[1], self.warping_layer.mask_mode, B)
        ops.corr81_norm_forward_c8(pair[0], pair[1], buf8[:, nconv:nconv + ncorr], leaky_slope=0.1)
        if not (use_sgu and FLOW16_IN_BLEND[0]):
            ops.flow_update_c8(flow_up, None, None, buf8[:, o_flow:o_flow + 1])
        res = est.forward_in_buffer_c8(buf8, in_map=in_map)
        ops.flow_update_c8(flow_up, res, None, buf8[:, o_flow + 1:o_flow + 2])
        nch = nconv * 8
        ctx_map = list(range(nch)) + [m + nch if m >= 0 else -1 for m in in_map] + [nch + 115, nch + 116] + [-1] * 6
        fine = self.context_networks.forward_c8(buf8, in_map=ctx_map)
        flow = ops.flow_update(flow_up, res, fine)
        self._tap('L%d.pair' % level, pair)
        self._tap('L%d.buf8' % level, buf8)
        self._tap('L%d.res' % level, res)
        self._tap('L%d.fine' % level, fine)
        return flow, [flow[:B], flow[B:]]

    def _level_update(self, Fn, Fwn, A, flow_up, add_to_flow=False):
        est = self.flow_estimators
        nb, _, H, W = Fn.shape
        nc = self.dim_corr
        fin = (lambda t: flow_up + t) if add_to_flow else (lambda t: t)
        if _fast_conv_ok(Fn):
            buf, slot = est.alloc_buffer(nb, H, W, Fn.dtype, Fn.device, tail=2)
            ops.corr81_forward_raw(Fn.contiguous(), Fwn.contiguous(), out=slot[:, :nc], leaky_slope=0.1)
            slot[:, nc:nc + 32] = A
            slot[:, nc + 32:] = flow_up
            x5, res = est.forward_in_buffer(buf)
            res = res.float()
            buf[:, est._n_total:] = flow_up + res
            fine = self.context_networks(buf).float()
            return fin(res + fine)
        if torch.is_grad_enabled() and (Fn.requires_grad or Fwn.requires_grad):
            c = self._corr_leaky(Fn, Fwn)
            if est.train_in_buffer_ok([c, A, flow_up]):
                buf, res = est.forward_train([c, A, flow_up], flow_tail=flow_up)
                fine = self.context_networks(buf)
                if add_to_flow and flow_up.dtype == torch.float32 and fine.dtype == res.dtype and res.dtype != torch.float32:
                    return ops.flow_sum3(flow_up, res, fine)
                return fin(res.float() + fine.float())
            x = torch.cat([c, A, flow_up.to(c.dtype)], dim=1)
        else:
            x = self._estimator_input(Fn, Fwn, A, flow_up)
        feat, res = est(x)
        res = res.float()
        fine = self.context_networks(torch.cat([feat, (flow_up + res).to(feat.dtype)], dim=1)).float()
        return fin(res + fine)

    def _corr_leaky(self, f_a, f_b_warp):
        c = self.correlation
        if (c.pad_size, c.kernel_size, c.max_displacement, c.stride1, c.stride2) == (4, 1, 4, 1, 1) and f_a.is_cuda:
            return ops.corr81(f_a, f_b_warp, float(self.leakyRELU.negative_slope))
        return self.leakyRELU(c(f_a, f_b_warp))

    def _estimator_input(self, f_a, f_b_warp, feat_1x1, flow):
        if torch.is_grad_enabled() and (f_a.requires_grad or f_b_warp.requires_grad):
            c = self._corr_leaky(f_a, f_b_warp)
            return torch.cat([c, feat_1x1, flow.to(c.dtype)], dim=1)
        B, _, H, W = f_a.shape
        buf = torch.empty((B, self.num_ch_in, H, W), dtype=f_a.dtype, device=f_a.device)
        ops.corr81_forward_raw(f_a.contiguous(), f_b_warp.contiguous(), out=buf[:, :self.dim_corr], leaky_slope=0.1)
        buf[:, self.dim_corr:self.dim_corr + 32] = feat_1x1
        buf[:, self.dim_corr + 32:] = flow
        return buf

    def decode_level_res(self, level, flow_1, flow_2, feature_1, feature_1_1x1, feature_2, feature_2_1x1, img_ori_1, img_ori_2):
        flow_1_up = upsample2d_flow_as(flow_1, feature_1, mode="bilinear", if_rate=True)
        flow_2_up = upsample2d_flow_as(flow_2, feature_2, mode="bilinear", if_rate=True)
        if level == 0:
            feature_2_warp, feature_1_warp = feature_2, feature_1
        else:
            if self.conf.if_sgu_upsample:
                flow_1_up = self.self_guided_upsample(flow_up_bilinear=flow_1_up, feature_1=feature_1_1x1, feature_2=feature_2_1x1)
                flow_2_up = self.self_guided_upsample(flow_up_bilinear=flow_2_up, feature_1=feature_2_1x1, feature_2=feature_1_1x1)
            feature_2_warp = self.warping_layer(feature_2, flow_1_up)
            feature_1_warp = self.warping_layer(feature_1, flow_2_up)
        if self.conf.if_norm_before_cost_volume:
            kw = dict(normalize=True, center=True, moments_across_channels=self.conf.norm_moments_across_channels,
                      moments_across_images=self.conf.norm_moments_across_images)
            feature_1, feature_2_warp = network_tools.normalize_features((feature_1, feature_2_warp), **kw)
            feature_2, feature_1_warp = network_tools.normalize_features((feature_2, feature_1_warp), **kw)
        in_1 = self._estimator_input(feature_1, feature_2_warp, feature_1_1x1, flow_1_up)
        in_2 = self._estimator_input(feature_2, feature_1_warp, feature_2_1x1, flow_2_up)
        feat_1, res_1 = self.flow_estimators(in_1)
        feat_2, res_2 = self.flow_estimators(in_2)
        res_1, res_2 = res_1.float(), res_2.float()
        fine_1 = self.context_networks(torch.cat([feat_1, (flow_1_up + res_1).to(feat_1.dtype)], dim=1)).float()
        fine_2 = self.context_networks(torch.cat([feat_2, (flow_2_up + res_2).to(feat_2.dtype)], dim=1)).float()
        return flow_1_up, flow_2_up, res_1 + fine_1, res_2 + fine_2

    def to_inference(self, dtype=torch.bfloat16, pyramid_dtype='auto', device=None):
        if device is not None:
            self.to(device)
        if isinstance(pyramid_dtype, str):
            if pyramid_dtype != 'auto':
                raise ValueError("to_inference: pyramid_dtype must be a torch dtype, None or 'auto'")
            pyramid_dtype = torch.float16 if dtype == torch.bfloat16 else None
        if pyramid_dtype is None or pyramid_dtype == dtype:
            return self.to(dtype).eval()
        if dtype not in (torch.bfloat16, torch.float16) or pyramid_dtype not in (torch.bfloat16, torch.float16):
            raise ValueError('to_inference: dtype / pyramid_dtype must be torch.bfloat16 or torch.float16')
        src = self.feature_pyramid_extractor.convs[0][0][0].weight.dtype
        if src != torch.float32:
            import warnings
            warnings.warn('to_inference(pyramid_dtype=...) on a network that is already %s: the pyramid keeps that rounding' % src)
        pyr = {id(m) for part in (self.feature_pyramid_extractor, self.conv_1x1) for m in part.modules()}
        for m in self.modules():
            for name, p_ in list(m._parameters.items()):
                if p_ is not None:
                    p_.data = p_.data.to(pyramid_dtype if id(m) in pyr else dtype)
        self.invalidate_packed()
        return self.eval()

    def froze_PWC(self):
        for part in (self.feature_pyramid_extractor, self.flow_estimators, self.context_networks, self.conv_1x1):
            for p in part.parameters():
                p.requires_grad = False

    def self_guided_upsample(self, flow_up_bilinear, feature_1, feature_2, output_level_flow=None):
        return self.sgi_model(flow_up_bilinear, feature_1, feature_2, output_level_flow=output_level_flow)[1]

    @classmethod
    def demo(cls, device='cuda'):
        conf = UPFlow_net.config()
        conf.update({'if_norm_before_cost_volume': True, 'norm_moments_across_channels': False,
                     'norm_moments_across_images': False, 'if_sgu_upsample': True})
        net = conf().to(device).eval()
        im = torch.rand(1, 3, 320, 320, device=device)
        with torch.no_grad():
            out = net({'im1': im, 'im2': im, 'if_loss': False})
        for k, v in out.items():
            tools.check_tensor(v, k)
```

upflow_pytorch_amd/ops.py:

```python
import os
import weakref

import torch
from torch.autograd import Function

from . import _lib
from ._lib import MASK_NONE, MASK_LITERAL, MASK_ROBUST, UpflowHipError

_MASKS = {None: MASK_NONE, 'none': MASK_NONE, 'literal': MASK_LITERAL, 'robust': MASK_ROBUST,
          MASK_NONE: MASK_NONE, MASK_LITERAL: MASK_LITERAL, MASK_ROBUST: MASK_ROBUST}


def _f32(t):
    return t if t.dtype == torch.float32 else t.float()


PITCH_MULTIPLE = 8


def empty_nchw(shape, dtype, device, pitched=True):
    W = shape[-1]
    if pitched and dtype in (torch.bfloat16, torch.float16) and W >= 8 and W % PITCH_MULTIPLE:
        Wp = (W + PITCH_MULTIPLE - 1) // PITCH_MULTIPLE * PITCH_MULTIPLE
        return torch.empty(tuple(shape[:-1]) + (Wp,), dtype=dtype, device=device)[..., :W]
# ... 490 lines not shown
        g_xo = torch.empty((B, 3, h, w), dtype=torch.float32, device=x_out.device)
        ws = torch.empty((_lib.lib().upf_sgu_blend_backward_workspace_bytes(B, h, w, Hf, Wf),), dtype=torch.uint8, device=x_out.device)
        with torch.cuda.device(dev):
            _lib.call('upf_sgu_blend_backward', _lib.ptr(flow_init), _lib.ptr(x_out), _lib.ptr(g_up), _lib.ptr(g_init),
                      _lib.ptr(g_xo), _lib.ptr(ws), B, h, w, Hf, Wf, _lib.dtype_code(x_out), _lib.stream_ptr(dev))
        return g_init, g_xo.to(x_out.dtype), None


def sgu_blend_flow16(flow_init, x_out, flow16):
    flow_init = _f32(flow_init).contiguous()
    x_out = x_out.contiguous()
    B, _, H, W = x_out.shape
    if tuple(flow_init.shape) != (B, 2, H, W) or x_out.shape[1] != 3 or x_out.dtype not in (torch.bfloat16, torch.float16) or flow16.dtype != x_out.dtype:
        raise UpflowHipError('sgu_blend_flow16: flow_init [B,2,H,W] fp32, x_out [B,3,H,W] 16-bit and a 16-bit flow slot of its type expected')
    c8 = flow16.dim() == 5
    if c8:
        if tuple(flow16.shape) != (B, 1, H, W, 8) or not _c8_view_ok(flow16):
            raise UpflowHipError('sgu_blend_flow16: the octet slot must be [B,1,H,W,8]')
    elif tuple(flow16.shape) != (B, 2, H, W) or not _is_channel_slice(flow16):
        raise UpflowHipError('sgu_blend_flow16: the NCHW slot must be a [B,2,H,W] channel slice of a contiguous buffer')
    dev = _lib.check_gpu(flow_init, x_out)
    flow_up = torch.empty_like(flow_init)
    with torch.cuda.device(dev):
        _lib.call('upf_sgu_blend_forward_flow16', _lib.ptr(flow_init), _lib.ptr(x_out), _lib.ptr(flow_up), _lib.ptr(flow16), flow16.stride(0), int(c8),
                  B, H, W, _lib.dtype_code(x_out), _lib.stream_ptr(dev))
    return flow_up


def sgu_blend(flow_init, x_out, output_level_flow=None, want_inter=True):
    base = output_level_flow if output_level_flow is not None else flow_init
    flow_up, inter_flow, inter_mask = SguBlendFunction.apply(base, x_out, want_inter)
    return base, flow_up, inter_flow, inter_mask


class NormalizeFunction(Function):
    @staticmethod
    def forward(ctx, x):
        x = x.contiguous()
        B, C, H, W = x.shape
        dev = _lib.check_gpu(x)
        y = torch.empty_like(x)
        rstd = torch.empty((B * C,), dtype=torch.float32, device=x.device)
        ws = torch.empty((_lib.lib().upf_normalize_workspace_bytes(B * C, H * W),), dtype=torch.uint8, device=x.device)
        with torch.cuda.device(dev):
            _lib.call('upf_normalize_forward', _lib.ptr(x), _lib.ptr(y), _lib.ptr(None), _lib.ptr(rstd), _lib.ptr(ws), B * C, H * W,
                      _lib.dtype_code(x), _lib.stream_ptr(dev))
        ctx.save_for_backward(y, rstd)
        return y

    @staticmethod
    def backward(ctx, gy):
        y, rstd = ctx.saved_tensors
        B, C, H, W = y.shape
        gy = gy.to(y.dtype).contiguous()
        dev = _lib.check_gpu(y, gy)
        gx = torch.empty_like(y)
        with torch.cuda.device(dev):
            _lib.call('upf_normalize_backward', _lib.ptr(y), _lib.ptr(gy), _lib.ptr(rstd), _lib.ptr(gx), B * C, H * W,
                      _lib.dtype_code(y), _lib.stream_ptr(dev))
        return gx


def normalize(x):
    return NormalizeFunction.apply(x)


def normalize_pair(a, b):
    return normalize(a), normalize(b)


def occ_check(flow_f, flow_b, alpha1=0.1, alpha2=0.5):
    ff = _f32(flow_f.detach()).contiguous()
    fb = _f32(flow_b.detach()).contiguous()
    B, _, H, W = ff.shape
    dev = _lib.check_gpu(ff, fb)
    o1 = torch.empty((B, 1, H, W), dtype=torch.float32, device=ff.device)
    o2 = torch.empty_like(o1)
    with torch.cuda.device(dev):
        _lib.call('upf_occ_check', _lib.ptr(ff), _lib.ptr(fb), _lib.ptr(o1), _lib.ptr(o2), B, H, W,
                  float(alpha1), float(alpha2), _lib.stream_ptr(dev))
    return o1, o2


CONV_X3_NPROD = [3]


def conv3x3_pack(weight):
    w = weight.detach().contiguous()
    Cout, Cin, kh, kw = w.shape
    if kh != kw or kh not in (1, 3):
        raise UpflowHipError('conv pack: 3x3 or 1x1 kernels only')
    dev = _lib.check_gpu(w)
    if w.dtype == torch.float32:
        packed = torch.empty((_lib.lib().upf_conv_x3_packed_bytes(Cin, Cout, kh) // 2,), dtype=torch.float16, device=w.device)
        with torch.cuda.device(dev):
            _lib.call('upf_conv_x3_pack_weights', _lib.ptr(w), _lib.ptr(packed), Cin, Cout, kh, _lib.stream_ptr(dev))
        return packed
    nbytes = _lib.lib().upf_conv_packed_bytes(Cin, Cout, kh)
    packed = torch.empty((nbytes // 2,), dtype=w.dtype, device=w.device)
    with torch.cuda.device(dev):
        _lib.call('upf_conv_pack_weights', _lib.ptr(w), _lib.ptr(packed), Cin, Cout, kh, _lib.dtype_code(w), _lib.stream_ptr(dev))
    return packed


def conv3x3_supported(x_view, Cout, dilation, stride=1, kernel_size=3):
    return (x_view.is_cuda and x_view.dtype in (torch.bfloat16, torch.float16, torch.float32) and kernel_size in (1, 3)
            and 1 <= dilation <= 16 and (stride == 1 or (stride == 2 and dilation == 1 and kernel_size == 3))
            and (x_view.shape[3] >= 8 or x_view.dtype == torch.float32))


def mfma_f16_denorm_probe(device):
    out = torch.zeros(1, dtype=torch.float32, device=device)
    with torch.cuda.device(device):
        _lib.call('upf_mfma_f16_denorm_probe', _lib.ptr(out), _lib.stream_ptr(device))
    return float(out.item()) == 2.0 ** -6


def conv_set_option(name, value):
    prev = _lib.lib().upf_conv_set_option(name.encode(), int(value))
    if prev == -2 ** 31:
        raise UpflowHipError('unknown convolution option %r' % name)
    return prev


def conv3x3_out_hw(H, W, stride=1):
    return (H - 1) // stride + 1, (W - 1) // stride + 1


def conv3x3_forward_raw(x_view, packed, bias32, y_view, dilation=1, leaky_slope=0.0, stride=1, kernel_size=3):
    B, Cin, H, W = x_view.shape
    Cout = y_view.shape[1]
    Ho, Wo = conv3x3_out_hw(H, W, stride)
    if tuple(y_view.shape) != (B, Cout, Ho, Wo):
        raise UpflowHipError('conv: output must be [%d,%d,%d,%d], got %s' % (B, Cout, Ho, Wo, tuple(y_view.shape)))
    xp, yp = _pitch_or_raise(x_view, 'conv: x'), _out_pitch_or_raise(y_view, 'conv: y')
    dev = x_view.device
    if x_view.dtype == torch.float32:
        if xp != W or yp != Wo:
            raise UpflowHipError('conv (fp32, split precision): contiguous rows expected (no row pitch)')
        if y_view.dtype != torch.float32 or packed.dtype != torch.float16:
            raise UpflowHipError('conv (fp32, split precision): fp32 output and weights packed from fp32 expected')
        with torch.cuda.device(dev):
            _lib.call('upf_conv_x3_forward', _lib.ptr(x_view), x_view.stride(0), _lib.ptr(packed), _lib.ptr(bias32),
                      _lib.ptr(y_view), y_view.stride(0), B, Cin, Cout, H, W, int(kernel_size), int(dilation), int(stride),
                      float(leaky_slope), int(CONV_X3_NPROD[0]), _lib.stream_ptr(dev))
        return y_view
    if y_view.dtype != x_view.dtype:
        if kernel_size != 1 or stride != 1 or Cout > 32 or y_view.dtype not in (torch.bfloat16, torch.float16):
            raise UpflowHipError('conv: an output type other than the operands\' is offered for 1x1 convolutions with Cout <= 32 only')
        with torch.cuda.device(dev):
            _lib.call('upf_conv1x1_forward_mixed', _lib.ptr(x_view), x_view.stride(0), xp, _lib.ptr(packed), _lib.ptr(bias32), _lib.ptr(y_view),
                      y_view.stride(0), yp, 0, B, Cin, Cout, H, W, float(leaky_slope), _lib.dtype_code(x_view), _lib.dtype_code(y_view), _lib.stream_ptr(dev))
        return y_view
    with torch.cuda.device(dev):
        _lib.call('upf_conv_forward_pitched', _lib.ptr(x_view), x_view.stride(0), xp, _lib.ptr(packed), _lib.ptr(bias32),
                  _lib.ptr(y_view), y_view.stride(0), yp, B, Cin, Cout, H, W, int(kernel_size), int(dilation), int(stride),
                  float(leaky_slope), _lib.dtype_code(x_view), _lib.stream_ptr(dev))
    return y_view


def conv3x3_forward_gated_raw(x_view, packed, bias32, y_view, add, act, mask_slope):
    B, Cin, H, W = x_view.shape
    Cout = y_view.shape[1]
    if tuple(y_view.shape) != (B, Cout, H, W):
        raise UpflowHipError('conv (gated): output must be [%d,%d,%d,%d], got %s' % (B, Cout, H, W, tuple(y_view.shape)))
    xp, yp = _pitch_or_raise(x_view, 'conv (gated): x'), _out_pitch_or_raise(y_view, 'conv (gated): y')
    if add is None and act is None:
        raise UpflowHipError('conv (gated): neither add nor act given')
    for t, name in ((add, 'add'), (act, 'act')):
        if t is None:
            continue
        if tuple(t.shape) != (B, Cout, H, W) or t.dtype != y_view.dtype or _pitch_or_raise(t, 'conv (gated): ' + name) != yp:
            raise UpflowHipError('conv (gated): %s must be a [%d,%d,%d,%d] channel slice of the output\'s dtype and row pitch' % (name, B, Cout, H, W))
    if x_view.dtype not in (torch.bfloat16, torch.float16) or y_view.dtype != x_view.dtype or not x_view.is_cuda:
        raise UpflowHipError('conv (gated): 16-bit GPU operands of one type expected (there is no CPU fallback)')
    dev = x_view.device
    with torch.cuda.device(dev):
        _lib.call('upf_conv_forward_gated', _lib.ptr(x_view), x_view.stride(0), xp, _lib.ptr(packed), _lib.ptr(bias32), _lib.ptr(y_view),
                  y_view.stride(0), yp, _lib.ptr(add), (add.stride(0) if add is not None else 0), _lib.ptr(act), (act.stride(0) if act is not None else 0),
                  float(mask_slope), B, Cin, Cout, H, W, _lib.dtype_code(x_view), _lib.stream_ptr(dev))
    return y_view


def c8_empty(B, C, H, W, dtype, device):
    return torch.empty((B, (C + 7) // 8, H, W, 8), dtype=dtype, device=device)


def to_c8(x):
    B, C, H, W = x.shape
    n = (C + 7) // 8
    if n * 8 != C:
        x = torch.cat([x, x.new_zeros(B, n * 8 - C, H, W)], 1)
    return x.view(B, n, 8, H, W).permute(0, 1, 3, 4, 2).contiguous()


def from_c8(x8, C=None):
    B, n, H, W, _ = x8.shape
    x = x8.permute(0, 1, 4, 2, 3).reshape(B, n * 8, H, W)
    return x if C is None else x[:, :C]


def conv_c8_k(n8_oct, C2):
    return _lib.lib().upf_conv_c8_k(int(n8_oct), int(C2))


def conv_c8_pack(weight, c8_channels=(), tail_channels=()):
    w = weight.detach().contiguous()
    Cout, Cin, kh, kw = w.shape
    if kh != kw or kh not in (1, 3):
        raise UpflowHipError('conv pack: 3x3 or 1x1 kernels only')
    c8_channels, tail_channels = list(c8_channels), list(tail_channels)
    if len(c8_channels) % 8:
        raise UpflowHipError('conv_c8_pack: the C8 slice must be whole octets')
    K = conv_c8_k(len(c8_channels) // 8, len(tail_channels))
    p8 = (len(c8_channels) + 31) // 32 * 32 if c8_channels else 0
    kmap = [-1] * K
    kmap[:len(c8_channels)] = c8_channels
    kmap[p8:p8 + len(tail_channels)] = tail_channels
    dev = _lib.check_gpu(w)
    kmap_t = torch.tensor(kmap, dtype=torch.int32, device=w.device)
    nbytes = _lib.lib().upf_conv_packed_bytes_k(K, Cout, kh)
    packed = torch.empty((nbytes // 2,), dtype=w.dtype, device=w.device)
    with torch.cuda.device(dev):
        _lib.call('upf_conv_pack_weights_kmap', _lib.ptr(w), _lib.ptr(packed), Cin, Cout, kh, _lib.ptr(kmap_t), K,
                  _lib.dtype_code(w), _lib.stream_ptr(dev))
    return packed


def conv_c8_narrow_ok(Cout, kernel_size, dilation, stride, has_tail):
    return Cout <= 16 and kernel_size == 3 and dilation == 1 and stride == 1 and not has_tail


def conv_c8_pack16(weight, c8_channels):
    w = weight.detach().contiguous()
    Cout, Cin, kh, kw = w.shape
    c8_channels = list(c8_channels)
    if kh != 3 or kw != 3 or len(c8_channels) % 8 or not c8_channels:
        raise UpflowHipError('conv_c8_pack16: 3x3 kernels, a C8 slice of whole octets')
    K = (len(c8_channels) + 31) // 32 * 32
    kmap = c8_channels + [-1] * (K - len(c8_channels))
    dev = _lib.check_gpu(w)
    kmap_t = torch.tensor(kmap, dtype=torch.int32, device=w.device)
    packed = torch.empty((_lib.lib().upf_conv_packed_bytes_k16(K, Cout) // 2,), dtype=w.dtype, device=w.device)
    with torch.cuda.device(dev):
        _lib.call('upf_conv_pack_weights_kmap16', _lib.ptr(w), _lib.ptr(packed), Cin, Cout, _lib.ptr(kmap_t), K,
                  _lib.dtype_code(w), _lib.stream_ptr(dev))
    return packed


def conv_c8_forward_narrow_raw(x8, packed16, bias32, y, leaky_slope=0.0):
    B, n, H, W, _ = x8.shape
    Cout = bias32.shape[0]
    y_is_c8 = y.dim() == 5
    if not _c8_view_ok(x8):
        raise UpflowHipError('conv_c8_narrow: x8 must be an octet slice of a contiguous C8 buffer')
    if y_is_c8:
        if not _c8_view_ok(y) or tuple(y.shape) != (B, (Cout + 7) // 8, H, W, 8):
            raise UpflowHipError('conv_c8_narrow: C8 output must be [%d,%d,%d,%d,8], got %s' % (B, (Cout + 7) // 8, H, W, tuple(y.shape)))
    elif tuple(y.shape) != (B, Cout, H, W) or y.stride()[1:] != (H * W, W, 1):
        raise UpflowHipError('conv_c8_narrow: NCHW output must be a [%d,%d,%d,%d] channel slice' % (B, Cout, H, W))
    dev = x8.device
    if not (x8.is_cuda and y.is_cuda) or x8.dtype != y.dtype:
        raise UpflowHipError('conv_c8_narrow: GPU tensors of one dtype expected (there is no CPU fallback)')
    with torch.cuda.device(dev):
        _lib.call('upf_conv_forward_c8_narrow', _lib.ptr(x8), x8.stride(0), n, _lib.ptr(packed16), _lib.ptr(bias32), _lib.ptr(y), y.stride(0),
                  int(y_is_c8), B, Cout, H, W, float(leaky_slope), _lib.dtype_code(x8), _lib.stream_ptr(dev))
    return y


def _partial_ok(partial, B, H, W):
    return (partial.dtype == torch.float32 and partial.dim() == 5 and partial.shape[0] == B and tuple(partial.shape[2:]) == (H, W, 4)
            and partial.stride()[1:] == (H * W * 4, W * 4, 4, 1))


def conv_c8_forward_split_raw(x8, packed, bias32, y8, partial, leaky_slope=0.0):
    B, n, H, W, _ = x8.shape
    Cout = bias32.shape[0]
    if not _c8_view_ok(x8) or not _c8_view_ok(y8) or tuple(y8.shape[0:1] + y8.shape[2:]) != (B, H, W, 8):
        raise UpflowHipError('conv_c8_split: x8 / y8 must be octet slices of contiguous C8 buffers of one size')
    cmain = 8 * y8.shape[1]
    if not _partial_ok(partial, B, H, W) or 4 * partial.shape[1] < (Cout - cmain + 3) // 4 * 4:
        raise UpflowHipError('conv_c8_split: partial must be fp32 [B,Q,H,W,4] (planes of channel quads, 4 Q >= the partial channels), got %s' % (tuple(partial.shape),))
    dev = x8.device
    if not (x8.is_cuda and y8.is_cuda and partial.is_cuda) or x8.dtype != y8.dtype:
        raise UpflowHipError('conv_c8_split: GPU tensors of one 16-bit dtype expected (there is no CPU fallback)')
    with torch.cuda.device(dev):
        _lib.call('upf_conv_forward_c8_split', _lib.ptr(x8), x8.stride(0), n, _lib.ptr(packed), _lib.ptr(bias32), _lib.ptr(y8), y8.stride(0), cmain,
                  _lib.ptr(partial), partial.stride(0), 4 * partial.shape[1], B, Cout, H, W, float(leaky_slope), _lib.dtype_code(x8), _lib.stream_ptr(dev))
    return y8


def conv_c8_forward_narrow_init_raw(x8, packed16, partial, offset, Cout, y, leaky_slope=0.0):
    B, n, H, W, _ = x8.shape
    y_is_c8 = y.dim() == 5
    if not _c8_view_ok(x8):
        raise UpflowHipError('conv_c8_narrow_init: x8 must be an octet slice of a contiguous C8 buffer')
    if y_is_c8:
        if not _c8_view_ok(y) or tuple(y.shape) != (B, (Cout + 7) // 8, H, W, 8):
            raise UpflowHipError('conv_c8_narrow_init: C8 output must be [%d,%d,%d,%d,8], got %s' % (B, (Cout + 7) // 8, H, W, tuple(y.shape)))
    elif tuple(y.shape) != (B, Cout, H, W) or y.stride()[1:] != (H * W, W, 1):
        raise UpflowHipError('conv_c8_narrow_init: NCHW output must be a [%d,%d,%d,%d] channel slice' % (B, Cout, H, W))
    if not _partial_ok(partial, B, H, W):
        raise UpflowHipError('conv_c8_narrow_init: partial must be fp32 [B,Q,H,W,4] (planes of channel quads)')
    dev = x8.device
    if not (x8.is_cuda and y.is_cuda and partial.is_cuda) or x8.dtype != y.dtype:
        raise UpflowHipError('conv_c8_narrow_init: GPU tensors of one 16-bit dtype expected (there is no CPU fallback)')
    with torch.cuda.device(dev):
        _lib.call('upf_conv_forward_c8_narrow_init', _lib.ptr(x8), x8.stride(0), n, _lib.ptr(packed16), _lib.ptr(partial), partial.stride(0), 4 * partial.shape[1],
                  int(offset), _lib.ptr(y), y.stride(0), int(y_is_c8), B, int(Cout), H, W, float(leaky_slope), _lib.dtype_code(x8), _lib.stream_ptr(dev))
    return y


def conv_pair_pack(w_a, w_b):
    C1, Cin, C2 = w_a.shape[0], w_a.shape[1], w_b.shape[0]
    if tuple(w_a.shape[2:]) != (3, 3) or tuple(w_b.shape[2:]) != (3, 3) or w_b.shape[1] != C1 or Cin > 16 or C1 not in (16, 32) or C2 > 32:
        raise UpflowHipError('conv_pair_pack: 3x3 layers with Cin <= 16, C1 = 16 | 32, C2 <= 32 expected, got %s / %s' % (tuple(w_a.shape), tuple(w_b.shape)))
    dev, dt = w_a.device, w_a.dtype
    lane = torch.arange(64, device=dev)
    co, kg, j = (lane % 32).view(1, 64, 1), (lane // 32).view(1, 64, 1), torch.arange(8, device=dev).view(1, 1, 8)
    wa = torch.zeros((32, 16, 12), dtype=dt, device=dev)
    wa[:C1, :Cin, :9] = w_a.detach().reshape(C1, Cin, 9)
    if Cin <= 4:
        s = torch.arange(3, device=dev).view(3, 1, 1)
        pa = wa[co.expand(3, 64, 8), (j % 4).expand(3, 64, 8), (4 * s + 2 * kg + j // 4).expand(3, 64, 8)]
    elif Cin <= 8:
        s = torch.arange(5, device=dev).view(5, 1, 1)
        pa = wa[co.expand(5, 64, 8), j.expand(5, 64, 8), (2 * s + kg).expand(5, 64, 8)]
    else:
        s = torch.arange(9, device=dev).view(9, 1, 1)
        pa = wa[co.expand(9, 64, 8), (8 * kg + j).expand(9, 64, 8), s.expand(9, 64, 8)]
    ksb = C1 // 16
    wbz = torch.zeros((32, C1, 9), dtype=dt, device=dev)
    wbz[:C2] = w_b.detach().reshape(C2, C1, 9)
    tap = torch.arange(9, device=dev).view(9, 1, 1, 1)
    ks = torch.arange(ksb, device=dev).view(1, ksb, 1, 1)
    shp = (9, ksb, 64, 8)
    pb = wbz[co.view(1, 1, 64, 1).expand(shp), (16 * ks + 8 * kg.view(1, 1, 64, 1) + j.view(1, 1, 1, 8)).expand(shp), tap.expand(shp)]
    return pa.contiguous(), pb.contiguous()


def conv_pair_forward_raw(x, packed_a, bias_a, slope_a, packed_b, bias_b, slope_b, y, strides=(1, 2)):
    B, Cin, H, W = x.shape
    C1, C2 = bias_a.shape[0], bias_b.shape[0]
    Ho, Wo = conv3x3_out_hw(H, W, 2)
    xp = _pitch_or_raise(x, 'conv_pair: x')
    y_is_c8 = y.dim() == 5
    if y_is_c8:
        if not _c8_view_ok(y) or tuple(y.shape) != (B, (C2 + 7) // 8, Ho, Wo, 8):
            raise UpflowHipError('conv_pair: C8 output must be [%d,%d,%d,%d,8], got %s' % (B, (C2 + 7) // 8, Ho, Wo, tuple(y.shape)))
        yp = 0
    else:
        if tuple(y.shape) != (B, C2, Ho, Wo):
            raise UpflowHipError('conv_pair: NCHW output must be [%d,%d,%d,%d], got %s' % (B, C2, Ho, Wo, tuple(y.shape)))
        yp = _out_pitch_or_raise(y, 'conv_pair: y')
    dev = x.device
    if not (x.is_cuda and y.is_cuda) or x.dtype != y.dtype or x.dtype not in (torch.bfloat16, torch.float16) or packed_a.dtype != x.dtype:
        raise UpflowHipError('conv_pair: GPU tensors of one 16-bit dtype expected (there is no CPU fallback)')
    with torch.cuda.device(dev):
        _lib.call('upf_conv_pair_forward', _lib.ptr(x), x.stride(0), xp, Cin, _lib.ptr(packed_a), _lib.ptr(bias_a), float(slope_a), C1, int(strides[0]),
                  _lib.ptr(packed_b), _lib.ptr(bias_b), float(slope_b), C2, int(strides[1]), _lib.ptr(y), y.stride(0), yp, int(y_is_c8), B, H, W,
                  _lib.dtype_code(x), _lib.stream_ptr(dev))
    return y


def conv_pair_supported(x, conv_a, conv_b):
    if torch.is_grad_enabled() or not x.is_cuda or x.dtype not in (torch.bfloat16, torch.float16) or x.dim() != 4:
        return False
    if (conv_a.stride, conv_b.stride) not in (((1, 1), (2, 2)), ((2, 2), (1, 1))):
        return False
    for c in (conv_a, conv_b):
        if c.kernel_size != (3, 3) or c.dilation != (1, 1) or c.padding != (1, 1) or c.groups != 1 or c.bias is None or c.weight.dtype != x.dtype:
            return False
    p = nchw_pitch(x)
    return (conv_a.in_channels <= 16 and conv_a.out_channels in (16, 32) and conv_b.in_channels == conv_a.out_channels and conv_b.out_channels <= 32
            and p is not None and p % 2 == 0 and x.data_ptr() % 4 == 0 and x.stride(0) % 2 == 0 and x.shape[3] >= 8)


def _c8_view_ok(t):
    B, n, H, W, e = t.shape
    return e == 8 and t.stride()[1:] == (H * W * 8, W * 8, 8, 1)


def conv_c8_supported(H, W, dtype, Cout, dilation, kernel_size, has_c8_in, has_tail, y_is_c8):
    if dtype not in (torch.bfloat16, torch.float16) or (W % 8 and has_tail):
        return False
    if kernel_size == 1:
        return (not has_c8_in) and has_tail and y_is_c8 and Cout <= 32
    if dilation == 1:
        return has_c8_in or (has_tail and y_is_c8)
    return dilation in (2, 4, 8, 16) and has_c8_in and not has_tail and y_is_c8


def conv_c8_forward_raw(x8, x2, packed, bias32, y, dilation=1, leaky_slope=0.0, kernel_size=3, stride=1):
    ref = x8 if x8 is not None else x2
    B, H, W = ref.shape[0], ref.shape[2], ref.shape[3]
    Cout = bias32.shape[0]
    y_is_c8 = y.dim() == 5
    Ho, Wo = conv3x3_out_hw(H, W, stride)
    if x8 is not None and not _c8_view_ok(x8):
        raise UpflowHipError('conv_c8: x8 must be an octet slice of a contiguous C8 buffer')
    x2p = _pitch_or_raise(x2, 'conv_c8: x2') if x2 is not None else 0
    yp = 0
    if y_is_c8:
        if not _c8_view_ok(y) or tuple(y.shape) != (B, (Cout + 7) // 8, Ho, Wo, 8):
            raise UpflowHipError('conv_c8: C8 output must be [%d,%d,%d,%d,8], got %s' % (B, (Cout + 7) // 8, Ho, Wo, tuple(y.shape)))
    else:
        if tuple(y.shape) != (B, Cout, Ho, Wo):
            raise UpflowHipError('conv_c8: NCHW output must be a [%d,%d,%d,%d] channel slice' % (B, Cout, Ho, Wo))
        yp = _out_pitch_or_raise(y, 'conv_c8: y')
    dev = ref.device
    if y.dtype != ref.dtype:
        if not (x8 is None and x2 is not None and kernel_size == 1 and stride == 1 and y_is_c8 and Cout <= 32 and y.dtype in (torch.bfloat16, torch.float16)):
            raise UpflowHipError('conv_c8: an output type other than the operands\' is offered for the 1x1 NCHW -> C8 projection (Cout <= 32) only')
        with torch.cuda.device(dev):
            _lib.call('upf_conv1x1_forward_mixed', _lib.ptr(x2), x2.stride(0), x2p, _lib.ptr(packed), _lib.ptr(bias32), _lib.ptr(y), y.stride(0), 0, 1,
                      B, x2.shape[1], Cout, H, W, float(leaky_slope), _lib.dtype_code(x2), _lib.dtype_code(y), _lib.stream_ptr(dev))
        return y
    with torch.cuda.device(dev):
        _lib.call('upf_conv_forward_c8_pitched', _lib.ptr(x8), x8.stride(0) if x8 is not None else 0, x8.shape[1] if x8 is not None else 0,
                  _lib.ptr(x2), x2.stride(0) if x2 is not None else 0, x2p, x2.shape[1] if x2 is not None else 0,
                  _lib.ptr(packed), _lib.ptr(bias32), _lib.ptr(y), y.stride(0), yp, int(y_is_c8), B, Cout, H, W, int(kernel_size),
                  int(dilation), int(stride), float(leaky_slope), _lib.dtype_code(ref), _lib.stream_ptr(dev))
    return y


def conv1x1_c8_dual_raw(x2, packed, bias32, y_a, y_b, leaky_slope=0.0):
    B, Cin, H, W = x2.shape
    Cout = bias32.shape[0]
    for y in (y_a, y_b):
        if y.dim() != 5 or not _c8_view_ok(y) or tuple(y.shape) != (B, (Cout + 7) // 8, H, W, 8) or y.dtype != y_a.dtype:
            raise UpflowHipError('conv1x1_c8_dual: outputs must be octet slices [%d,%d,%d,%d,8] of one type' % (B, (Cout + 7) // 8, H, W))
    xp = _pitch_or_raise(x2, 'conv1x1_c8_dual: x')
    dev = x2.device
    if not (x2.is_cuda and y_a.is_cuda and y_b.is_cuda) or x2.dtype not in (torch.bfloat16, torch.float16) or y_a.dtype not in (torch.bfloat16, torch.float16):
        raise UpflowHipError('conv1x1_c8_dual: 16-bit GPU tensors expected (there is no CPU fallback)')
    with torch.cuda.device(dev):
        _lib.call('upf_conv1x1_forward_c8_dual', _lib.ptr(x2), x2.stride(0), xp, _lib.ptr(packed), _lib.ptr(bias32), _lib.ptr(y_a), y_a.stride(0),
                  _lib.ptr(y_b), y_b.stride(0), B, Cin, Cout, H, W, float(leaky_slope), _lib.dtype_code(x2), _lib.dtype_code(y_a), _lib.stream_ptr(dev))
    return y_a


def conv_c8_set_option(name, value):
    prev = _lib.lib().upf_conv_c8_set_option(name.encode(), int(value))
    if prev == -2 ** 31:
        raise UpflowHipError('unknown C8 convolution option %r' % name)
    return prev


def conv_x3_set_option(name, value):
    prev = _lib.lib().upf_conv_x3_set_option(name.encode(), int(value))
    if prev == -2 ** 31:
        raise UpflowHipError('unknown split-precision convolution option %r' % name)
    return prev


class CensusFunction(Function):
    @staticmethod
    def forward(ctx, gray1, gray2, max_distance):
        gray1 = _f32(gray1).contiguous()
        gray2 = _f32(gray2).contiguous()
        if gray1.dim() != 4 or gray1.shape[1] != 1 or gray1.shape != gray2.shape:
            raise UpflowHipError('census: two [B,1,H,W] grey images expected, got %s / %s' % (tuple(gray1.shape), tuple(gray2.shape)))
        B, _, H, W = gray1.shape
        dev = _lib.check_gpu(gray1, gray2)
        dist = torch.empty_like(gray1)
        with torch.cuda.device(dev):
            _lib.call('upf_census_forward', _lib.ptr(gray1), _lib.ptr(gray2), _lib.ptr(dist), B, H, W, int(max_distance), _lib.stream_ptr(dev))
        ctx.save_for_backward(gray1, gray2)
        ctx.max_distance = int(max_distance)
        return dist

    @staticmethod
    def backward(ctx, g):
        gray1, gray2 = ctx.saved_tensors
        B, _, H, W = gray1.shape
        g = _f32(g).contiguous()
        dev = _lib.check_gpu(gray1, gray2, g)
        g1 = torch.empty_like(gray1) if ctx.needs_input_grad[0] else None
        g2 = torch.empty_like(gray2) if ctx.needs_input_grad[1] else None
        if g1 is None and g2 is None:
            return None, None, None
        with torch.cuda.device(dev):
            _lib.call('upf_census_backward', _lib.ptr(gray1), _lib.ptr(gray2), _lib.ptr(g), _lib.ptr(g1), _lib.ptr(g2), B, H, W,
                      ctx.max_distance, _lib.stream_ptr(dev))
        return g1, g2, None


def census_distance(gray1, gray2, max_distance=3):
    return CensusFunction.apply(gray1, gray2, max_distance)


class BoundaryWarpFunction(Function):
    @staticmethod
    def forward(ctx, image, flow, start):
        image = _f32(image).contiguous()
        flow = _f32(flow).contiguous()
        B, C, Hi, Wi = image.shape
        if flow.dim() != 4 or flow.shape[0] != B or flow.shape[1] != 2:
            raise UpflowHipError('boundary_warp: image [B,C,Hi,Wi] and flow [B,2,h,w] expected, got %s / %s' % (tuple(image.shape), tuple(flow.shape)))
        start = _f32(start).to(flow.device).reshape(-1)
        if start.numel() == 2:
            start = start.repeat(B)
        if start.numel() != 2 * B:
            raise UpflowHipError('boundary_warp: start must hold (x, y) per batch item, got %d values for B=%d' % (start.numel(), B))
        start = start.contiguous()
        h, w = flow.shape[2:]
        dev = _lib.check_gpu(image, flow, start)
        out = torch.empty((B, C, h, w), dtype=torch.float32, device=flow.device)
        with torch.cuda.device(dev):
            _lib.call('upf_boundary_warp_forward', _lib.ptr(image), _lib.ptr(flow), _lib.ptr(start), _lib.ptr(out), B, C, Hi, Wi, h, w,
                      _lib.stream_ptr(dev))
        ctx.save_for_backward(image, flow, start)
        return out

    @staticmethod
    def backward(ctx, g):
        image, flow, start = ctx.saved_tensors
        if ctx.needs_input_grad[0]:
            raise UpflowHipError('boundary_warp: the gradient wrt the image is not implemented (frames are data)')
        B, C, Hi, Wi = image.shape
        h, w = flow.shape[2:]
        g = _f32(g).contiguous()
        dev = _lib.check_gpu(image, flow, g)
        gflow = torch.empty_like(flow)
        with torch.cuda.device(dev):
            _lib.call('upf_boundary_warp_backward', _lib.ptr(image), _lib.ptr(flow), _lib.ptr(start), _lib.ptr(g), _lib.ptr(gflow),
                      B, C, Hi, Wi, h, w, _lib.stream_ptr(dev))
        return None, gflow, None


def boundary_warp(image, flow, start):
    return BoundaryWarpFunction.apply(image, flow, start)


class RobustLossFunction(Function):
    @staticmethod
    def forward(ctx, x, y, occ, q, eps):
        x = _f32(x).contiguous()
        y = _f32(y).contiguous()
        if x.shape != y.shape or x.dim() != 4:
            raise UpflowHipError('robust_loss: two [B,C,H,W] tensors expected, got %s / %s' % (tuple(x.shape), tuple(y.shape)))
        B, C, H, W = x.shape
        if occ is not None:
            occ = _f32(occ).contiguous()
            if tuple(occ.shape) != (B, 1, H, W):
                raise UpflowHipError('robust_loss: occlusion mask must be [B,1,H,W], got %s' % (tuple(occ.shape),))
        dev = _lib.check_gpu(x, y, occ)
        nb = _lib.lib().upf_loss_partials(B * H * W)
        partials = torch.empty((nb, 2), dtype=torch.float32, device=x.device)
        with torch.cuda.device(dev):
            _lib.call('upf_robust_loss_forward', _lib.ptr(x), _lib.ptr(y), _lib.ptr(occ), _lib.ptr(partials), B, C, H * W, float(eps), float(q),
                      _lib.stream_ptr(dev))
        sums = partials.sum(0)
        ctx.save_for_backward(x, y, occ)
        ctx.qe = (float(q), float(eps))
        s_loss, s_occ = sums.unbind(0)
        ctx.mark_non_differentiable(s_occ)
        ctx.set_materialize_grads(False)
        return s_loss, s_occ

    @staticmethod
    def backward(ctx, g, _g_occ):
        if g is None:
            return None, None, None, None, None
        if len(ctx.needs_input_grad) > 2 and ctx.needs_input_grad[2]:
            raise UpflowHipError('robust_loss: the occlusion weights are treated as constants (hard masks); a mask that '
                                 'requires grad would silently get a zero gradient')
        x, y, occ = ctx.saved_tensors
        q, eps = ctx.qe
        B, C, H, W = x.shape
        coef = _f32(g).reshape(1).contiguous()
        dev = _lib.check_gpu(x, y, coef)
        gx = torch.empty_like(x) if ctx.needs_input_grad[0] else None
        gy = torch.empty_like(y) if ctx.needs_input_grad[1] else None
        if gx is None and gy is None:
            return None, None, None, None, None
        with torch.cuda.device(dev):
            _lib.call('upf_robust_loss_backward', _lib.ptr(x), _lib.ptr(y), _lib.ptr(occ), _lib.ptr(coef), _lib.ptr(gx), _lib.ptr(gy),
                      B, C, H * W, eps, q, _lib.stream_ptr(dev))
        return gx, gy, None, None, None


def robust_loss_sums(x, y, occ=None, q=0.4, eps=0.01):
    return RobustLossFunction.apply(x, y, occ, q, eps)


def grey(image):
    image = _f32(image).contiguous()
    B, C, H, W = image.shape
    if C != 3:
        raise UpflowHipError('grey: an RGB image [B,3,H,W] expected, got %s' % (tuple(image.shape),))
    dev = _lib.check_gpu(image)
    out = torch.empty((B, 1, H, W), dtype=torch.float32, device=image.device)
    with torch.cuda.device(dev):
        _lib.call('upf_grey_forward', _lib.ptr(image), _lib.ptr(out), B, H * W, _lib.stream_ptr(dev))
    return out


class MsdUpupFunction(Function):

    @staticmethod
    def forward(ctx, y, occ, weight, q, eps, *levels):
        y = _f32(y).contiguous()
        B, C, H, W = y.shape
        if C != 2 or not levels or len(levels) > 6:
            raise UpflowHipError('msd_upup: a [B,2,H,W] label and 1..6 level flows expected')
        xs = [_f32(x).contiguous() for x in levels]
        for x in xs:
            if x.dim() != 4 or x.shape[0] != B or x.shape[1] != 2:
                raise UpflowHipError('msd_upup: level flows must be [B,2,h,w], got %s' % (tuple(x.shape),))
        if occ is not None:
            occ = _f32(occ).contiguous()
            if tuple(occ.shape) != (B, 1, H, W):
                raise UpflowHipError('msd_upup: occlusion mask must be [B,1,H,W], got %s' % (tuple(occ.shape),))
            if occ.requires_grad:
                raise UpflowHipError('msd_upup: the occlusion weights are treated as constants (hard masks)')
        dev = _lib.check_gpu(y, occ, *xs)
        n = len(xs)
        nb = _lib.lib().upf_msd_upup_partials(B, H, W)
        partials = torch.empty((nb, 7), dtype=torch.float32, device=y.device)
        out2 = torch.empty((2,), dtype=torch.float32, device=y.device)
        xp = (_lib._vp * n)(*[x.data_ptr() for x in xs])
        hs = (_lib._c.c_int * n)(*[x.shape[2] for x in xs])
        ws = (_lib._c.c_int * n)(*[x.shape[3] for x in xs])
        with torch.cuda.device(dev):
            _lib.call('upf_msd_upup_forward', xp, hs, ws, n, _lib.ptr(y), _lib.ptr(occ), _lib.ptr(partials), _lib.ptr(out2), B, H, W,
                      float(weight), float(eps), float(q), _lib.stream_ptr(dev))
        ctx.save_for_backward(y, occ, out2, *xs)
        ctx.cfg = (float(weight), float(q), float(eps))
        ctx.set_materialize_grads(False)
        return out2[0]

    @staticmethod
    def backward(ctx, g):
        n = len(ctx.saved_tensors) - 3
        if g is None:
            return (None,) * (5 + n)
        y, occ, out2 = ctx.saved_tensors[:3]
        xs = ctx.saved_tensors[3:]
        weight, q, eps = ctx.cfg
        B, _, H, W = y.shape
        g = _f32(g).reshape(1).contiguous()
        dev = _lib.check_gpu(y, g)
        gxs = [torch.empty_like(x) for x in xs]
        xp = (_lib._vp * n)(*[x.data_ptr() for x in xs])
        gp = (_lib._vp * n)(*[x.data_ptr() for x in gxs])
        hs = (_lib._c.c_int * n)(*[x.shape[2] for x in xs])
        ws = (_lib._c.c_int * n)(*[x.shape[3] for x in xs])
        with torch.cuda.device(dev):
            _lib.call('upf_msd_upup_backward', xp, gp, hs, ws, n, _lib.ptr(y), _lib.ptr(occ), _lib.ptr(g), _lib.ptr(out2), B, H, W,
                      weight, eps, q, _lib.stream_ptr(dev))
        return (None, None, None, None, None) + tuple(gx if ctx.needs_input_grad[5 + i] else None for i, gx in enumerate(gxs))


def msd_upup_supported(y, levels):
    return (y.is_cuda and y.dim() == 4 and y.shape[1] == 2 and 1 <= len(levels) <= 6 and y.shape[2] > 1 and y.shape[3] > 1
            and all(x.is_cuda and x.dim() == 4 and x.shape[1] == 2 and 2 <= x.shape[3] <= y.shape[3] and 1 <= x.shape[2] <= y.shape[2]
                    and (y.shape[3] - 1) / (x.shape[3] - 1) <= 250 for x in levels))


def msd_upup_loss(levels, y, occ=None, weight=1.0, q=0.4, eps=0.01):
    return MsdUpupFunction.apply(y, occ, weight, q, eps, *levels)


class SmoothEdge1Function(Function):
    @staticmethod
    def forward(ctx, img, pred):
        img = _f32(img).contiguous()
        pred = _f32(pred).contiguous()
        if img.dim() != 4 or pred.dim() != 4 or img.shape[0] != pred.shape[0] or img.shape[2:] != pred.shape[2:]:
            raise UpflowHipError('smooth_edge1: img [B,Ci,H,W] and pred [B,Cp,H,W] expected, got %s / %s' % (tuple(img.shape), tuple(pred.shape)))
        B, Ci, H, W = img.shape
        Cp = pred.shape[1]
        if H < 2 or W < 2:
            raise UpflowHipError('smooth_edge1: at least 2x2 pixels')
        dev = _lib.check_gpu(img, pred)
        nb = _lib.lib().upf_loss_partials(B * H * W)
        partials = torch.empty((nb, 2), dtype=torch.float32, device=img.device)
# ... 740 lines not shown
```

Baseline: 1915 frame-pairs/s.

## Ingest fp32 frames directly in the first fused conv pair, skipping stack/cast copies

Adds an fp32-input variant of the fused conv-pair kernel. It reads the two raw frame batches through separate base pointers and converts them to bf16/fp16 while loading into LDS. The model routes the first feature-pyramid stage and the SGU guidance stem through this path, so the concatenate-and-cast copies of the input frames are no longer needed. In exchange, the kernel reads twice as many input bytes and gains a branch on the batch index for choosing the base pointer.

Measured after the change: 1929 frame-pairs/s (median of 6 runs). No clear change (+0.7%).

```diff
diff --git a/include/upflow_hip.h b/include/upflow_hip.h
--- a/include/upflow_hip.h
+++ b/include/upflow_hip.h
@@ -163,6 +163,12 @@
                           const void* wb_packed, const float* bias_b , float slope_b, int C2, int stride_b,
                           void* y, long long y_batch_stride, int y_row_pitch, int y_is_c8,
                           int B, int H, int W, int dtype, void* stream);
+
+int upf_conv_pair_forward_f32(const float* x1, const float* x2, int B1, long long x_batch_stride, int x_row_pitch, int Cin,
+                              const void* wa_packed, const float* bias_a , float slope_a, int C1, int stride_a,
+                              const void* wb_packed, const float* bias_b , float slope_b, int C2, int stride_b,
+                              void* y, long long y_batch_stride, int y_row_pitch, int y_is_c8,
+                              int B, int H, int W, int dtype, void* stream);
 
 int upf_conv_pack_weights_f32(const float* w , void* w_packed, int Cin, int Cout, int kernel_size,
                               int dtype, int dgrad, void* stream);
diff --git a/upflow_pytorch_amd/_lib.py b/upflow_pytorch_amd/_lib.py
--- a/upflow_pytorch_amd/_lib.py
+++ b/upflow_pytorch_amd/_lib.py
@@ -64,6 +64,7 @@
     'upf_conv_forward_c8_split': [_vp, _ll, _i, _vp, _vp, _vp, _ll, _i, _vp, _ll, _i, _i, _i, _i, _i, _f, _i, _vp],
     'upf_conv_forward_c8_narrow_init': [_vp, _ll, _i, _vp, _vp, _ll, _i, _i, _vp, _ll, _i, _i, _i, _i, _i, _f, _i, _vp],
     'upf_conv_pair_forward': [_vp, _ll, _i, _i, _vp, _vp, _f, _i, _i, _vp, _vp, _f, _i, _i, _vp, _ll, _i, _i, _i, _i, _i, _i, _vp],
+    'upf_conv_pair_forward_f32': [_vp, _vp, _i, _ll, _i, _i, _vp, _vp, _f, _i, _i, _vp, _vp, _f, _i, _i, _vp, _ll, _i, _i, _i, _i, _i, _i, _vp],
     'upf_leaky_backward': [_vp, _vp, _vp, _ll, _f, _i, _vp],
     'upf_conv_wgrad': [_vp, _ll, _vp, _ll, _vp, _vp, _i, _i, _i, _i, _i, _i, _i, _i, _vp],
     'upf_conv_bias_grad': [_vp, _ll, _vp, _vp, _i, _i, _i, _i, _vp],
diff --git a/upflow_pytorch_amd/csrc/conv_pair.hip b/upflow_pytorch_amd/csrc/conv_pair.hip
--- a/upflow_pytorch_amd/csrc/conv_pair.hip
+++ b/upflow_pytorch_amd/csrc/conv_pair.hip
@@ -14,9 +14,9 @@
   static constexpr int IR = SA * (MR - 1) + 3, IC = (SA * (MC - 1) + 3 + XO + 1) / 2 * 2;
 };
 
-template <typename T, int K0, int C1O, int TH, bool YC8, int SA, int SB>
+template <typename T, int K0, int C1O, int TH, bool YC8, int SA, int SB, bool F32IN>
 __global__ __launch_bounds__(NT, 2)
-void conv_pair_kernel(const T* __restrict__ x, long long xbs, int xpitch, int Cin, const T* __restrict__ wa, const float* __restrict__ ba, float slope_a,
+void conv_pair_kernel(const void* __restrict__ x, const void* __restrict__ x2, int nsplit, long long xbs, int xpitch, int Cin, const T* __restrict__ wa, const float* __restrict__ ba, float slope_a,
                       const T* __restrict__ wb, const float* __restrict__ bb, float slope_b, T* __restrict__ y, long long ybs, int ypitch, int C2,
                       int H, int W, int Hm, int Wm, int Ho, int Wo, int tiles_x, int tiles_y) {
   using G = Geo<SA, SB, TH>;
@@ -38,19 +38,30 @@
   const int px = lane & 31, kg = lane >> 5;
 
   {
-    const uint32_t plane = (uint32_t)(H * xpitch) * 2u;
-    __amdgpu_buffer_rsrc_t xr = __builtin_amdgcn_make_buffer_rsrc(const_cast<T*>(x + (size_t)n * xbs), 0, (uint32_t)Cin * plane, 0x00020000);
+    static_assert(!F32IN || QUAD, "fp32 ingest: the frames (Cin <= 4)");
+    constexpr uint32_t ES = F32IN ? 4u : 2u;
+    const uint32_t plane = (uint32_t)(H * xpitch) * ES;
+    const unsigned char* xn = (F32IN && n >= nsplit) ? static_cast<const unsigned char*>(x2) + (size_t)(n - nsplit) * xbs * ES
+                                                     : static_cast<const unsigned char*>(x) + (size_t)n * xbs * ES;
+    __amdgpu_buffer_rsrc_t xr = __builtin_amdgcn_make_buffer_rsrc(const_cast<unsigned char*>(xn), 0, (uint32_t)Cin * plane, 0x00020000);
     const int iy0 = SA * my0 - 1, ix0 = SA * mx0 - 1 - XO;
     for (int item = tid; item < IR * (IC / 2); item += NT) {
       const int ir = item / (IC / 2), pp = item - ir * (IC / 2);
       const int gy = iy0 + ir, gx = ix0 + 2 * pp;
       const bool in = gy >= 0 && gy < H && gx >= 0 && gx < W;
-      const uint32_t off = in ? (uint32_t)(gy * xpitch + gx) * 2u : 0x80000000u;
+      const uint32_t off = in ? (uint32_t)(gy * xpitch + gx) * ES : 0x80000000u;
       const uint32_t hm = (gx + 1 < W) ? 0xffffffffu : 0x0000ffffu;
       if constexpr (QUAD) {
         uint32_t ch[4];
 #pragma unroll
-        for (int c = 0; c < 4; ++c) ch[c] = __builtin_amdgcn_raw_buffer_load_b32(xr, off + (uint32_t)c * plane, 0, 0) & hm;
+        for (int c = 0; c < 4; ++c) {
+          if constexpr (F32IN) {
+            const u32x2 f2 = __builtin_amdgcn_raw_buffer_load_b64(xr, off + (uint32_t)c * plane, 0, 0);
+            ch[c] = pack2<T>(__uint_as_float(f2.x), __uint_as_float(f2.y)) & hm;
+          } else {
+            ch[c] = __builtin_amdgcn_raw_buffer_load_b32(xr, off + (uint32_t)c * plane, 0, 0) & hm;
+          }
+        }
         uint2 e0, e1;
         e0.x = __builtin_amdgcn_perm(ch[1], ch[0], 0x05040100u); e1.x = __builtin_amdgcn_perm(ch[1], ch[0], 0x07060302u);
         e0.y = __builtin_amdgcn_perm(ch[3], ch[2], 0x05040100u); e1.y = __builtin_amdgcn_perm(ch[3], ch[2], 0x07060302u);
@@ -201,12 +212,12 @@
 }
 
 struct PairArgs {
-  const void* x; long long xbs; int xpitch, Cin; const void* wa; const float* ba; float slope_a; int C1;
+  const void* x; const void* x2; int nsplit; long long xbs; int xpitch, Cin; const void* wa; const float* ba; float slope_a; int C1;
   const void* wb; const float* bb; float slope_b; int C2; void* y; long long ybs; int ypitch; int B, H, W; hipStream_t stream;
   int sa, sb;
 };
 
-template <typename T, int K0, int C1O, int TH, bool YC8, int SA, int SB>
+template <typename T, int K0, int C1O, int TH, bool YC8, int SA, int SB, bool F32IN = false>
 int launch_pair(const PairArgs& a) {
   using G = Geo<SA, SB, TH>;
   const int Hm = (a.H - 1) / SA + 1, Wm = (a.W - 1) / SA + 1;
@@ -214,9 +225,9 @@
   const int tiles_x = cdiv(Wo, 32), tiles_y = cdiv(Ho, TH);
   const size_t ldsb = (size_t)((K0 == 0 ? (G::IR * G::IC + 1) / 2 : K0 * G::IR * G::IC) + C1O * G::MR * G::MC) * 16;
   static LdsOptIn opt;
-  auto kern = &conv_pair_kernel<T, K0, C1O, TH, YC8, SA, SB>;
+  auto kern = &conv_pair_kernel<T, K0, C1O, TH, YC8, SA, SB, F32IN>;
   opt.ensure(reinterpret_cast<const void*>(kern), ldsb);
-  hipLaunchKernelGGL(kern, dim3((unsigned)(a.B * tiles_x * tiles_y)), dim3(NT), ldsb, a.stream, (const T*)a.x, a.xbs, a.xpitch, a.Cin,
+  hipLaunchKernelGGL(kern, dim3((unsigned)(a.B * tiles_x * tiles_y)), dim3(NT), ldsb, a.stream, a.x, a.x2, a.nsplit, a.xbs, a.xpitch, a.Cin,
                      (const T*)a.wa, a.ba, a.slope_a, (const T*)a.wb, a.bb, a.slope_b, (T*)a.y, a.ybs, a.ypitch, a.C2, a.H, a.W, Hm, Wm, Ho, Wo, tiles_x, tiles_y);
   return check_launch("conv_pair_forward");
 }
@@ -224,6 +235,12 @@
 template <typename T, bool YC8>
 int dispatch_pair(const PairArgs& a) {
   const int k0 = a.Cin <= 4 ? 0 : (a.Cin <= 8 ? 1 : 2), c1o = a.C1 / 8;
+  if (a.x2) {
+    if (a.sa == 1) return c1o == 2 ? launch_pair<T, 0, 2, 8, YC8, 1, 2, true>(a) : launch_pair<T, 0, 4, 4, YC8, 1, 2, true>(a);
+    if constexpr (!YC8) return c1o == 2 ? launch_pair<T, 0, 2, 8, false, 2, 1, true>(a) : launch_pair<T, 0, 4, 8, false, 2, 1, true>(a);
+    set_error("conv_pair_forward_f32: [stride 2, stride 1] writes NCHW");
+    return UPF_EUNSUPPORTED;
+  }
   if (a.sa == 1) {
     if (k0 == 0 && c1o == 2) return launch_pair<T, 0, 2, 8, YC8, 1, 2>(a);
     if (k0 == 0 && c1o == 4) return launch_pair<T, 0, 4, 4, YC8, 1, 2>(a);
@@ -271,8 +288,37 @@
   UPF_REQUIRE(aligned_to(wa_packed, 16) && aligned_to(wb_packed, 16), UPF_EINVAL, "conv_pair_forward: packed weights must be 16-byte aligned");
   UPF_REQUIRE(y_is_c8 ? (aligned_to(y, 16) && y_batch_stride % 8 == 0) : (y_row_pitch >= Wo), UPF_EINVAL, "conv_pair_forward: bad output layout");
   UPF_REQUIRE((long long)Cin * H * x_row_pitch * 2 < (1ll << 31), UPF_EINVAL, "conv_pair_forward: image too large for one buffer descriptor");
-  convp::PairArgs a{x, x_batch_stride, x_row_pitch, Cin, wa_packed, bias_a, slope_a == 0.f ? 1.f : slope_a, C1,
+  convp::PairArgs a{x, nullptr, 0, x_batch_stride, x_row_pitch, Cin, wa_packed, bias_a, slope_a == 0.f ? 1.f : slope_a, C1,
                     wb_packed, bias_b, slope_b == 0.f ? 1.f : slope_b, C2, y, y_batch_stride, y_row_pitch, B, H, W, (hipStream_t)stream, stride_a, stride_b};
   if (dtype == UPF_BF16) return y_is_c8 ? convp::dispatch_pair<bf16_t, true>(a) : convp::dispatch_pair<bf16_t, false>(a);
   return y_is_c8 ? convp::dispatch_pair<f16_t, true>(a) : convp::dispatch_pair<f16_t, false>(a);
 }
+
+extern "C" int upf_conv_pair_forward_f32(const float* x1, const float* x2, int B1, long long x_batch_stride, int x_row_pitch, int Cin,
+                                         const void* wa_packed, const float* bias_a, float slope_a, int C1, int stride_a,
+                                         const void* wb_packed, const float* bias_b, float slope_b, int C2, int stride_b,
+                                         void* y, long long y_batch_stride, int y_row_pitch, int y_is_c8,
+                                         int B, int H, int W, int dtype, void* stream) {
+  using namespace upf;
+  UPF_REQUIRE(x1 && x2 && wa_packed && bias_a && wb_packed && bias_b && y, UPF_EINVAL, "conv_pair_forward_f32: null pointer");
+  UPF_REQUIRE(B > 0 && H > 0 && W > 0 && B1 >= 0 && B1 <= B, UPF_EINVAL, "conv_pair_forward_f32: bad shape B=%d (first %d from x1) H=%d W=%d", B, B1, H, W);
+  UPF_REQUIRE(dtype == UPF_BF16 || dtype == UPF_F16, UPF_EDTYPE, "conv_pair_forward_f32: bf16 / fp16 compute only");
+  UPF_REQUIRE(Cin >= 1 && Cin <= 4 && (C1 == 16 || C1 == 32) && C2 >= 1 && C2 <= 32, UPF_EUNSUPPORTED,
+              "conv_pair_forward_f32: Cin <= 4, C1 = 16 | 32, C2 <= 32 (got %d, %d, %d)", Cin, C1, C2);
+  UPF_REQUIRE((stride_a == 1 && stride_b == 2) || (stride_a == 2 && stride_b == 1), UPF_EUNSUPPORTED,
+              "conv_pair_forward_f32: strides (1, 2) or (2, 1), got (%d, %d)", stride_a, stride_b);
+  UPF_REQUIRE(!(y_is_c8 && stride_a == 2), UPF_EUNSUPPORTED, "conv_pair_forward_f32: [stride 2, stride 1] writes NCHW");
+  if (x_row_pitch == 0) x_row_pitch = W;
+  const int Wo = (W - 1) / 2 + 1;
+  if (y_row_pitch == 0) y_row_pitch = Wo;
+  UPF_REQUIRE(x_row_pitch >= W && x_row_pitch % 2 == 0 && aligned_to(x1, 8) && aligned_to(x2, 8) && x_batch_stride % 2 == 0, UPF_EUNSUPPORTED,
+              "conv_pair_forward_f32: the input rows are read as fp32 pixel pairs: an even row pitch (%d) and 8-byte aligned bases", x_row_pitch);
+  UPF_REQUIRE(slope_a >= 0.f && slope_a <= 1.f && slope_b >= 0.f && slope_b <= 1.f, UPF_EINVAL, "conv_pair_forward_f32: leaky slopes in [0,1]");
+  UPF_REQUIRE(aligned_to(wa_packed, 16) && aligned_to(wb_packed, 16), UPF_EINVAL, "conv_pair_forward_f32: packed weights must be 16-byte aligned");
+  UPF_REQUIRE(y_is_c8 ? (aligned_to(y, 16) && y_batch_stride % 8 == 0) : (y_row_pitch >= Wo), UPF_EINVAL, "conv_pair_forward_f32: bad output layout");
+  UPF_REQUIRE((long long)Cin * H * x_row_pitch * 4 < (1ll << 31), UPF_EINVAL, "conv_pair_forward_f32: image too large for one buffer descriptor");
+  convp::PairArgs a{x1, x2, B1, x_batch_stride, x_row_pitch, Cin, wa_packed, bias_a, slope_a == 0.f ? 1.f : slope_a, C1,
+                    wb_packed, bias_b, slope_b == 0.f ? 1.f : slope_b, C2, y, y_batch_stride, y_row_pitch, B, H, W, (hipStream_t)stream, stride_a, stride_b};
+  if (dtype == UPF_BF16) return y_is_c8 ? convp::dispatch_pair<bf16_t, true>(a) : convp::dispatch_pair<bf16_t, false>(a);
+  return y_is_c8 ? convp::dispatch_pair<f16_t, true>(a) : convp::dispatch_pair<f16_t, false>(a);
+}
diff --git a/upflow_pytorch_amd/model/pwc_modules.py b/upflow_pytorch_amd/model/pwc_modules.py
--- a/upflow_pytorch_amd/model/pwc_modules.py
+++ b/upflow_pytorch_amd/model/pwc_modules.py
@@ -85,6 +85,15 @@
         cache = self.__dict__.setdefault('_fast_cache', {})
         hip = getattr(self, 'hip_convs', True)
         for i, stage in enumerate(self.convs):
+            if isinstance(x, _Frames32):
+                if i != 0 or not self.takes_frames(x):
+                    raise ops.UpflowHipError('FeatureExtractor: fp32 frame ingest without an eligible first stage')
+                pc = cache.get(('pair', i)) or cache.setdefault(('pair', i), _PackedConvPair(stage[0], stage[1]))
+                ho, wo = ops.conv3x3_out_hw(x.shape[2], x.shape[3], 2)
+                y = outs[i] if (outs is not None and outs[i] is not None) else ops.empty_nchw((x.shape[0], stage[1][0].out_channels, ho, wo), x.dtype, x.device, pitched=pitched)
+                x = pc(x, y)
+                pyramid.append(x)
+                continue
             if (hip and FUSE_PAIRS[0] and not getattr(self, '_no_fuse_pairs', False) and len(stage[0]) == 2 and len(stage[1]) == 2
                     and ops.conv_pair_supported(x, stage[0][0], stage[1][0])):
                 pc = cache.get(('pair', i)) or cache.setdefault(('pair', i), _PackedConvPair(stage[0], stage[1]))
@@ -97,6 +106,11 @@
             x = fast_conv_seq(stage[1], x, cache, out=None if outs is None else outs[i], allow_hip=hip, pitched=pitched)
             pyramid.append(x)
         return pyramid[::-1]
+
+    def takes_frames(self, frames):
+        stage = self.convs[0]
+        return (getattr(self, 'hip_convs', True) and frames_direct_enabled() and not getattr(self, '_no_fuse_pairs', False)
+                and len(stage[0]) == 2 and len(stage[1]) == 2 and ops.conv_pair_f32_supported(frames.x1, frames.x2, frames.dtype, stage[0][0], stage[1][0]))
 
     def out_shapes(self, H, W):
         shapes = []
@@ -369,12 +383,36 @@
 
     def __call__(self, x, y):
         pa, ba, pb, bb = self.get()
+        if isinstance(x, _Frames32):
+            return ops.conv_pair_forward_f32_raw(x.x1, x.x2, pa, ba, self.slopes[0], pb, bb, self.slopes[1], y, self.strides)
         return ops.conv_pair_forward_raw(x, pa, ba, self.slopes[0], pb, bb, self.slopes[1], y, self.strides)
+
+
+class _Frames32(object):
+
+    def __init__(self, x1, x2, dtype):
+        self.x1, self.x2, self.dtype = x1, x2, dtype
+        self.shape = torch.Size((2 * x1.shape[0],) + tuple(x1.shape[1:]))
+        self.device, self.is_cuda = x1.device, x1.is_cuda
+
+    def size(self):
+        return self.shape
+
+    def dim(self):
+        return 4
+
+    def as_dtype(self, dtype):
+        return self if dtype == self.dtype else _Frames32(self.x1, self.x2, dtype)
 
 
 DUAL_1X1 = [True]
 FUSE_PAIRS = [True]
 MERGE_TAIL = [True]
+FRAMES_DIRECT = [True]
+
+
+def frames_direct_enabled():
+    return FRAMES_DIRECT[0] and FUSE_PAIRS[0]
 
 
 def c8_level_ok(nb, H, W, dtype):
diff --git a/upflow_pytorch_amd/model/upflow.py b/upflow_pytorch_amd/model/upflow.py
--- a/upflow_pytorch_amd/model/upflow.py
+++ b/upflow_pytorch_amd/model/upflow.py
@@ -71,6 +71,21 @@
             cache = self.__dict__.setdefault('_fast_cache', {})
             n = len(self.upsample_output_conv)
             from . import pwc_modules as _pm
+            if isinstance(x, _pm._Frames32):
+                if not self.takes_frames(x):
+                    raise ops.UpflowHipError('SGU guidance stem: fp32 frame ingest without the two fused pairs')
+                sq = self.upsample_output_conv
+                B_, _, H_, W_ = x.shape
+                h1, w1 = ops.conv3x3_out_hw(H_, W_, 2)
+                mid = ops.empty_nchw((B_, sq[1][0].out_channels, h1, w1), x.dtype, x.device, pitched=True)
+                pa = cache.get('pair01') or cache.setdefault('pair01', _pm._PackedConvPair(sq[0], sq[1]))
+                pb = cache.get('pair23') or cache.setdefault('pair23', _pm._PackedConvPair(sq[2], sq[3]))
+                pa(x, mid)
+                h2, w2 = ops.conv3x3_out_hw(h1, w1, 2)
+                if out8 is not None:
+                    return pb(mid, out8)
+                y = out if out is not None else ops.empty_nchw((B_, sq[3][0].out_channels, h2, w2), x.dtype, x.device, pitched=pitched)
+                return pb(mid, y)
             if n == 4 and _pm.FUSE_PAIRS[0] and not getattr(self, '_no_fuse_pairs', False) and all(len(q) == 2 for q in self.upsample_output_conv):
                 sq = self.upsample_output_conv
                 if ops.conv_pair_supported(x, sq[0][0], sq[1][0]):
@@ -94,6 +109,15 @@
                     return pc(None, x, out8)
                 x = fast_conv_seq(seq, x, cache, out=out if i == n - 1 else None, pitched=pitched)
             return x
+
+        def takes_frames(self, frames):
+            from . import pwc_modules as _pm
+            sq = self.upsample_output_conv
+            if not (len(sq) == 4 and _pm.frames_direct_enabled() and not getattr(self, '_no_fuse_pairs', False) and all(len(q) == 2 for q in sq)):
+                return False
+            w1 = ops.conv3x3_out_hw(frames.shape[2], frames.shape[3], 2)[1]
+            return (ops.conv_pair_f32_supported(frames.x1, frames.x2, frames.dtype, sq[0][0], sq[1][0])
+                    and ops.conv_pair_layers_ok(frames.dtype, sq[2][0], sq[3][0]) and w1 >= 8)
 
     @classmethod
     def normalize_features(cls, feature_list, normalize, center, moments_across_channels=True, moments_across_images=True):
@@ -341,11 +365,14 @@
     def _forward_2_frame_v3(self, x1_raw, x2_raw, if_loss, cdt):
         if not torch.is_grad_enabled() or getattr(self, 'stacked_training', True):
             B = x1_raw.shape[0]
+            ddt = self.flow_estimators.conv1[0].weight.dtype
+            frames = self._frames_direct(x1_raw, x2_raw, cdt, ddt)
+            if frames is not None:
+                return self._forward_stacked_fast(frames, B, None if ddt == cdt else frames.as_dtype(ddt))
             X = ops.empty_nchw((2 * B,) + tuple(x1_raw.shape[1:]), cdt, x1_raw.device,
                                pitched=self._pitched() and not torch.is_grad_enabled() and x1_raw.is_cuda)
             X[:B].copy_(x1_raw)
             X[B:].copy_(x2_raw)
-            ddt = self.flow_estimators.conv1[0].weight.dtype
             if ddt != cdt:
                 if torch.is_grad_enabled() or not x1_raw.is_cuda or ddt == torch.float32 or cdt == torch.float32:
                     raise ops.UpflowHipError('pyramid_dtype: 16-bit GPU inference only')
@@ -386,9 +413,7 @@
 
     def _forward_stacked(self, X, B, train_dtype=None, frames_dec=None):
 
-        if (_fast_conv_ok(X) and X.dtype != torch.float32 and self.conf.if_norm_before_cost_volume and not self.conf.norm_moments_across_channels
-                and not self.conf.norm_moments_across_images and not getattr(self, '_no_fast_stacked', False)
-                and self.feature_pyramid_extractor.out_shapes(X.shape[2], X.shape[3])[-1][2] >= 8):
+        if self._takes_fast_stacked(X):
             return self._forward_stacked_fast(X, B, frames_dec)
         ddt = None if frames_dec is None else frames_dec.dtype
         pyramid = self.feature_pyramid_extractor(X)
@@ -429,6 +454,24 @@
             flow_out = self.sgi_model(flow, G, G, output_level_flow=flow_out, batch_shift=B)[1]
         f_out, b_out = ops.split_batch(flow_out, B)
         return f_out, b_out, flows[::-1]
+
+    def _takes_fast_stacked(self, X):
+        return (_fast_conv_ok(X) and X.dtype != torch.float32 and self.conf.if_norm_before_cost_volume and not self.conf.norm_moments_across_channels
+                and not self.conf.norm_moments_across_images and not getattr(self, '_no_fast_stacked', False)
+                and self.feature_pyramid_extractor.out_shapes(X.shape[2], X.shape[3])[-1][2] >= 8)
+
+    def _frames_direct(self, x1_raw, x2_raw, cdt, ddt):
+        from .pwc_modules import _Frames32, frames_direct_enabled
+        if (not frames_direct_enabled() or getattr(self, '_no_frames_direct', False) or torch.is_grad_enabled() or getattr(self, '_taps', None) is not None
+                or x1_raw.dim() != 4 or x1_raw.dtype != torch.float32 or x2_raw.dtype != torch.float32 or not x1_raw.is_cuda
+                or cdt not in (torch.bfloat16, torch.float16) or ddt not in (torch.bfloat16, torch.float16)):
+            return None
+        frames = _Frames32(x1_raw, x2_raw, cdt)
+        if not self._takes_fast_stacked(frames) or not self.feature_pyramid_extractor.takes_frames(frames):
+            return None
+        if self.conf.if_sgu_upsample and not self.sgi_model.takes_frames(frames.as_dtype(ddt)):
+            return None
+        return frames
 
     def _pitched(self):
         return not getattr(self, '_no_pitch', False)
diff --git a/upflow_pytorch_amd/ops.py b/upflow_pytorch_amd/ops.py
--- a/upflow_pytorch_amd/ops.py
+++ b/upflow_pytorch_amd/ops.py
@@ -816,6 +816,9 @@
         raise UpflowHipError('conv_c8_narrow_init: NCHW output must be a [%d,%d,%d,%d] channel slice' % (B, Cout, H, W))
     if not _partial_ok(partial, B, H, W):
         raise UpflowHipError('conv_c8_narrow_init: partial must be fp32 [B,Q,H,W,4] (planes of channel quads)')
+    if int(offset) < 0 or int(offset) % 4 or not 1 <= int(Cout) <= 16 or int(offset) + (int(Cout) + 3) // 4 * 4 > 4 * partial.shape[1]:
+        raise UpflowHipError('conv_c8_narrow_init: Cout <= 16 partial channels [%d, %d) must start at a quad and lie (whole quads) inside the %d partial channels'
+                             % (offset, int(offset) + int(Cout), 4 * partial.shape[1]))
     dev = x8.device
     if not (x8.is_cuda and y.is_cuda and partial.is_cuda) or x8.dtype != y.dtype:
         raise UpflowHipError('conv_c8_narrow_init: GPU tensors of one 16-bit dtype expected (there is no CPU fallback)')
@@ -877,17 +880,67 @@
     return y
 
 
-def conv_pair_supported(x, conv_a, conv_b):
-    if torch.is_grad_enabled() or not x.is_cuda or x.dtype not in (torch.bfloat16, torch.float16) or x.dim() != 4:
+def conv_pair_layers_ok(dtype, conv_a, conv_b):
+    if dtype not in (torch.bfloat16, torch.float16):
         return False
     if (conv_a.stride, conv_b.stride) not in (((1, 1), (2, 2)), ((2, 2), (1, 1))):
         return False
     for c in (conv_a, conv_b):
-        if c.kernel_size != (3, 3) or c.dilation != (1, 1) or c.padding != (1, 1) or c.groups != 1 or c.bias is None or c.weight.dtype != x.dtype:
+        if c.kernel_size != (3, 3) or c.dilation != (1, 1) or c.padding != (1, 1) or c.groups != 1 or c.bias is None or c.weight.dtype != dtype:
             return False
+    return conv_a.in_channels <= 16 and conv_a.out_channels in (16, 32) and conv_b.in_channels == conv_a.out_channels and conv_b.out_channels <= 32
+
+
+def conv_pair_supported(x, conv_a, conv_b):
+    if torch.is_grad_enabled() or not x.is_cuda or x.dtype not in (torch.bfloat16, torch.float16) or x.dim() != 4:
+        return False
+    if not conv_pair_layers_ok(x.dtype, conv_a, conv_b):
+        return False
     p = nchw_pitch(x)
-    return (conv_a.in_channels <= 16 and conv_a.out_channels in (16, 32) and conv_b.in_channels == conv_a.out_channels and conv_b.out_channels <= 32
-            and p is not None and p % 2 == 0 and x.data_ptr() % 4 == 0 and x.stride(0) % 2 == 0 and x.shape[3] >= 8)
+    return p is not None and p % 2 == 0 and x.data_ptr() % 4 == 0 and x.stride(0) % 2 == 0 and x.shape[3] >= 8
+
+
+def conv_pair_f32_supported(x1, x2, dtype, conv_a, conv_b):
+    if torch.is_grad_enabled() or x1.dim() != 4 or x1.shape != x2.shape or x1.stride() != x2.stride():
+        return False
+    if not (x1.is_cuda and x2.is_cuda) or x1.device != x2.device or x1.dtype != torch.float32 or x2.dtype != torch.float32:
+        return False
+    if not conv_pair_layers_ok(dtype, conv_a, conv_b) or conv_a.in_channels > 4 or conv_a.in_channels != x1.shape[1]:
+        return False
+    p = nchw_pitch(x1)
+    return (p is not None and p % 2 == 0 and x1.data_ptr() % 8 == 0 and x2.data_ptr() % 8 == 0 and x1.stride(0) % 2 == 0 and x1.shape[3] >= 8
+            and x1.shape[1] * x1.shape[2] * p * 4 < 2 ** 31)
+
+
+def conv_pair_forward_f32_raw(x1, x2, packed_a, bias_a, slope_a, packed_b, bias_b, slope_b, y, strides=(1, 2)):
+    if x1.dim() != 4 or x1.shape != x2.shape or x1.stride() != x2.stride():
+        raise UpflowHipError('conv_pair_f32: two [B,Cin,H,W] frame batches of one shape and one layout expected, got %s %s / %s %s'
+                             % (tuple(x1.shape), tuple(x1.stride()), tuple(x2.shape), tuple(x2.stride())))
+    B1, Cin, H, W = x1.shape
+    B = 2 * B1
+    C1, C2 = bias_a.shape[0], bias_b.shape[0]
+    Ho, Wo = conv3x3_out_hw(H, W, 2)
+    xp = _pitch_or_raise(x1, 'conv_pair_f32: x')
+    if Cin > 4 or xp % 2 or x1.data_ptr() % 8 or x2.data_ptr() % 8 or x1.stride(0) % 2:
+        raise UpflowHipError('conv_pair_f32: Cin <= 4, an even row pitch and 8-byte aligned frames expected (Cin %d, pitch %d)' % (Cin, xp))
+    y_is_c8 = y.dim() == 5
+    if y_is_c8:
+        if not _c8_view_ok(y) or tuple(y.shape) != (B, (C2 + 7) // 8, Ho, Wo, 8):
+            raise UpflowHipError('conv_pair_f32: C8 output must be [%d,%d,%d,%d,8], got %s' % (B, (C2 + 7) // 8, Ho, Wo, tuple(y.shape)))
+        yp = 0
+    else:
+        if tuple(y.shape) != (B, C2, Ho, Wo):
+            raise UpflowHipError('conv_pair_f32: NCHW output must be [%d,%d,%d,%d], got %s' % (B, C2, Ho, Wo, tuple(y.shape)))
+        yp = _out_pitch_or_raise(y, 'conv_pair_f32: y')
+    dev = y.device
+    if (not (x1.is_cuda and x2.is_cuda and y.is_cuda) or x1.device != dev or x2.device != dev or x1.dtype != torch.float32 or x2.dtype != torch.float32
+            or y.dtype not in (torch.bfloat16, torch.float16) or packed_a.dtype != y.dtype or packed_b.dtype != y.dtype):
+        raise UpflowHipError('conv_pair_f32: fp32 GPU frames and a 16-bit GPU output of the packed weights\' type expected (there is no CPU fallback)')
+    with torch.cuda.device(dev):
+        _lib.call('upf_conv_pair_forward_f32', _lib.ptr(x1), _lib.ptr(x2), B1, x1.stride(0), xp, Cin, _lib.ptr(packed_a), _lib.ptr(bias_a), float(slope_a), C1,
+                  int(strides[0]), _lib.ptr(packed_b), _lib.ptr(bias_b), float(slope_b), C2, int(strides[1]), _lib.ptr(y), y.stride(0), yp, int(y_is_c8),
+                  B, H, W, _lib.dtype_code(y), _lib.stream_ptr(dev))
+    return y
 
 
 def _c8_view_ok(t):
```
